# ronin-gw/PyMaSC

Measured on AMD Instinct MI355X. Metric: shifts*genome-bp/sec (whole node), hg38 max_shift=1000; HBM-BW fraction, higher is better.
Workload: dtype u64

## Files before the change

### pymasc_amd/csrc/kernels_events.h

```cpp
#pragma once

#define EV_NQ 2u
#define EV_TBW (EV_NQ * SP_TBW)
#define EV_TB (EV_NQ * SP_TB)
#define EV_LO 64u
#define EV_LO_MAX 512u
#define EV_HI 36u
#ifndef EV_CAPF
#define EV_CAPF 768u
#endif
#ifndef EV_CAPR
#define EV_CAPR 1000u
#endif
#ifndef EV_CAPE_SMALL
#define EV_CAPE_SMALL 1536u
#endif
#define EV_CAPE(BIG) ((BIG) ? 384u : EV_CAPE_SMALL)
#ifndef EV_POOL_SMALL
#define EV_POOL_SMALL 2416u
#endif
#define EV_POOL_ENTRIES(HAS_M, BIG) ((BIG) ? EV_CAPF + EV_CAPR + ((HAS_M) ? 384u : 0u) : ((HAS_M) ? EV_POOL_SMALL : EV_CAPF + EV_CAPR + EV_CAPE_SMALL))
#define EV_RANK_BITS 13u
#ifndef EV_POOL_DEEP
#define EV_POOL_DEEP 4328u
#endif
#define EV_POS 0x1ffffu
#define EV_PAD 12u
#define EV_RSENT 0x3fffffffu
#define EV_JOBSUM(jobstat) (reinterpret_cast<unsigned long long *>((jobstat) + 4 * SP_MAXJOBS))
#define EV_STAT_BYTES (4 * SP_MAXJOBS * sizeof(u32) + 6 * SP_MAXJOBS * sizeof(unsigned long long))
#define EV_SEG_ROWS 6u
#define EV_MAX_SHIFT 8191u
#ifndef EV_PRIO_STAGE
#define EV_PRIO_STAGE 3
#endif
#ifndef EV_PRIO_EVENTS
#define EV_PRIO_EVENTS 2
#endif
#ifndef EV_PRIO_EDGES
#define EV_PRIO_EDGES 1
#endif
#ifndef EV_EDGE_ROLES
#define EV_EDGE_ROLES 1
#endif
#ifndef EV_PAIR_SLOT
#define EV_PAIR_SLOT(w) (w)
#endif
#ifndef EV_ROLE_F
#define EV_ROLE_F 1
#define EV_ROLE_A 2
#define EV_ROLE_B0 3
#define EV_ROLE_B1 0
#endif
#ifndef EV_WAVES
#define EV_WAVES 5
#endif
#ifndef EV_WAVES_NCC
#define EV_WAVES_NCC 8
#endif

#ifdef EV_STAMPS
#define EV_NSTAMP 12
#define EV_STAMP(i)                                                                                    \
    {                                                                                                  \
        unsigned long long t_;                                                                         \
        __builtin_amdgcn_sched_barrier(0);                                                             \
        asm volatile("s_memtime %0\n\ts_waitcnt lgkmcnt(0)" : "=s"(t_)::"memory");                     \
        __builtin_amdgcn_sched_barrier(0);                                                             \
        stamp_acc[i] += t_ - stamp_last;                                                               \
        stamp_last = t_;                                                                               \
    }
#else
#define EV_STAMP(i)
#endif

template <bool HAS_M, bool BIG, bool DEEP = false>
struct EvLds {
    static constexpr u32 LF = 0;
    static constexpr u32 POOL = DEEP ? EV_POOL_DEEP : EV_POOL_ENTRIES(HAS_M, BIG);
    static_assert(POOL + 3 * EV_PAD < (1u << EV_RANK_BITS), "rank field of the forward entries");
    static constexpr u32 WT = LF + POOL + 3 * EV_PAD;
    static constexpr u32 MISC = WT + 32;
    static constexpr u32 IDXF = MISC + 16;
    static constexpr u32 IDXR = IDXF + (HAS_M ? 66u : 0u);
    static constexpr u32 MT0 = IDXR + (HAS_M ? 66u : 0u);
    static_assert(MT0 % 4 == 0, "alignment of the 16-byte stores");
    __host__ __device__ static constexpr u32 sg_words(u32 lo, u32 hi = EV_HI) { return MT0 + (HAS_M ? 4u + lo + EV_TBW + hi : 0u); }
    __host__ __device__ static constexpr u32 row_words(u32 hn) { return BIG ? hn / 2 : hn; }
    __host__ __device__ static constexpr u32 o_gf(u32 hn) { return hn; }
    __host__ __device__ static constexpr u32 o_gr(u32 hn) { return o_gf(hn) + (HAS_M ? row_words(hn) : 0u); }
    __host__ __device__ static constexpr u32 o_ee(u32 hn) { return o_gf(hn); }
    __host__ __device__ static constexpr u32 o_dump(u32 hn) { return o_gr(hn) + (HAS_M ? row_words(hn) : 0u); }
    __host__ __device__ static constexpr u32 o_xch(u32 hn) { return o_dump(hn) + 64; }
    __host__ __device__ static constexpr u32 o_sg(u32 hn) { return o_xch(hn) + 16; }
    __host__ __device__ static constexpr u32 total(u32 hn, u32 lo, u32 nsg, u32 hi = EV_HI) { return o_sg(hn) + nsg * sg_words(lo, hi); }
};

struct EvRegs {
    uint4 f[EV_NQ], r[EV_NQ], m[EV_NQ], h;
    u32 wb[EV_NQ], hbw;
};

template <bool BIG>
__device__ __forceinline__ bool ev_role_mlo(u32 tid, u32 lo) { return BIG ? tid < (lo >> 2) : (tid >> 6) == 1 && (tid & 63u) < 16; }
template <bool BIG>
__device__ __forceinline__ u32 ev_role_mlo_index(u32 tid) { return BIG ? tid : (tid & 63u); }

#ifndef EV_BIG_NT
#define EV_BIG_NT 1
#endif
typedef u32 ev_v4u __attribute__((ext_vector_type(4)));
template <bool GUARD, bool NT>
__device__ __forceinline__ uint4 ev_ld_body(const u32 *__restrict__ p, int64_t j, uint64_t nbits)
{
    if (GUARD || !NT) return ld_quad<GUARD>(p, j, nbits);
    const ev_v4u v = __builtin_nontemporal_load(reinterpret_cast<const ev_v4u *>(p + j));
    return make_uint4(v.x, v.y, v.z, v.w);
}

template <bool HAS_M, bool GUARD, bool BIG>
__device__ __forceinline__ void ev_fetch(EvRegs &er, const u32 *__restrict__ F, const u32 *__restrict__ R,
                                         const u32 *__restrict__ M, int64_t d0, uint64_t nbits, u32 tid, u32 nhr, u32 lo,
                                         bool skip_reads, u32 nhm = EV_HI / 4u)
{
    if (skip_reads) nhr = 0;
#pragma unroll
    for (u32 q = 0; q < EV_NQ; q++) {
        const int64_t j = d0 + (int64_t)q * SP_TBW + 4 * (int64_t)tid;
        if (skip_reads) {
            er.f[q] = make_uint4(0, 0, 0, 0);
            er.r[q] = make_uint4(0, 0, 0, 0);
        } else {
            er.f[q] = ev_ld_body<GUARD, BIG && EV_BIG_NT>(F, j, nbits);
            er.r[q] = ev_ld_body<GUARD, BIG && EV_BIG_NT>(R, j, nbits);
        }
        if (HAS_M) {
            er.m[q] = ev_ld_body<GUARD, BIG && EV_BIG_NT>(M, j, nbits);
            const int64_t j0 = d0 + (int64_t)q * SP_TBW + 4 * (int64_t)(tid & ~63u) - 1;
            er.wb[q] = GUARD ? ld_dword_guarded(M, j0, nbits) : M[j0];
        } else {
            er.m[q] = make_uint4(0, 0, 0, 0);
            er.wb[q] = 0;
        }
    }
    const u32 ht = tid & 63u, hw = tid >> 6;
    const bool m_lo = HAS_M && ev_role_mlo<BIG>(tid, lo), m_hi = HAS_M && hw == 2 && ht < nhm, r_hi = hw == 3 && ht < nhr;
    const u32 *hp = (m_lo || m_hi || skip_reads) ? M : R;
    int64_t jh = d0 + 4 * (int64_t)tid;
    if (m_lo) jh = d0 - (int64_t)lo + 4 * (int64_t)ev_role_mlo_index<BIG>(tid);
    if (m_hi || r_hi) jh = d0 + EV_TBW + 4 * (int64_t)ht;
    er.h = ld_quad<GUARD>(hp, jh, nbits);
    er.hbw = 0;
    if (HAS_M) {
        const bool lo_wave = BIG ? hw < 2 : hw == 1;
        const int64_t jh0 = (lo_wave ? d0 - (int64_t)lo + (BIG ? 256 * (int64_t)hw : 0) : d0 + EV_TBW) - 1;
        er.hbw = GUARD ? ld_dword_guarded(M, jh0, nbits) : M[jh0];
    }
}

template <bool HAS_M>
__device__ __forceinline__ void ev_fetch_fast(EvRegs &er, const SpJobRegs &jb, u32 local_tile, u32 tid, u32 wave, u32 nhr)
{
    const size_t tb = (size_t)local_tile * (EV_TBW * 4u);
    const char *fb = reinterpret_cast<const char *>(jb.F) + tb;
    const char *rb = reinterpret_cast<const char *>(jb.R) + tb;
    const char *mb = reinterpret_cast<const char *>(jb.M) + tb;
    const u32 voff = 16u * tid, lane = tid & 63u;
#pragma unroll
    for (u32 q = 0; q < EV_NQ; q++) {
        const u32 vq = voff + q * (SP_TBW * 4u);
        er.f[q] = *reinterpret_cast<const uint4 *>(fb + vq);
        er.r[q] = *reinterpret_cast<const uint4 *>(rb + vq);
        if (HAS_M) {
            er.m[q] = *reinterpret_cast<const uint4 *>(mb + vq);
            const int32_t sq = (int32_t)(q * (SP_TBW * 4u) + wave * 1024u) - 4;
            er.wb[q] = *reinterpret_cast<const u32 *>(mb + sq);
        } else {
            er.m[q] = make_uint4(0, 0, 0, 0);
            er.wb[q] = 0;
        }
    }
    const char *hb = (HAS_M && wave == 1) ? mb - EV_LO * 4u : (HAS_M && wave == 2) ? mb + EV_TBW * 4u : wave == 3 ? rb + EV_TBW * 4u : rb;
    const u32 lim = (HAS_M && wave == 1) ? 63u : (HAS_M && wave == 2) ? 8u : wave == 3 ? nhr - 1u : 63u;
    const u32 vh = 16u * (lane < lim ? lane : lim);
    er.h = *reinterpret_cast<const uint4 *>(hb + vh);
    er.hbw = HAS_M ? *reinterpret_cast<const u32 *>(hb - 4) : 0u;
}

template <bool HAS_M, bool BIG>
__device__ __forceinline__ void ev_fetch_job(EvRegs &er, const SpJobRegs &jb, u32 local_tile, u32 tid, u32 nhr, u32 lo,
                                             bool skip_reads = false, u32 wave = 0, u32 hi_dwords = EV_HI)
{
    const int64_t d0 = (int64_t)local_tile * EV_TBW;
    const int64_t low = d0 - (int64_t)lo - 1;
    const u32 above = (BIG && 4 * nhr > hi_dwords) ? 4 * nhr : hi_dwords;
    const uint64_t hi = (uint64_t)d0 + EV_TBW + above;
    const bool interior = jb.aligned16 && low >= 0 && hi + 2 <= jb.nbits / 32;
#ifndef EV_NO_FAST_FETCH
    if (!BIG && interior && !skip_reads)
        ev_fetch_fast<HAS_M>(er, jb, local_tile, tid, wave, nhr);
    else
#endif
    if (interior)
        ev_fetch<HAS_M, false, BIG>(er, jb.F, jb.R, jb.M, d0, jb.nbits, tid, nhr, lo, skip_reads, hi_dwords / 4u);
    else
        ev_fetch<HAS_M, true, BIG>(er, jb.F, jb.R, jb.M, d0, jb.nbits, tid, nhr, lo, skip_reads, hi_dwords / 4u);
}

__device__ __forceinline__ void ev_emit_f(const uint4 f, const uint4 r, const uint4 m, u32 idx, u32 rank0, u32 base_bit,
                                          u32 *list)
{
    const u64 fs[2] = {(u64)f.x | ((u64)f.y << 32), (u64)f.z | ((u64)f.w << 32)};
    const u64 rs[2] = {(u64)r.x | ((u64)r.y << 32), (u64)r.z | ((u64)r.w << 32)};
    const u64 ms[2] = {(u64)m.x | ((u64)m.y << 32), (u64)m.z | ((u64)m.w << 32)};
    u32 rk = rank0;
#pragma unroll
    for (u32 k = 0; k < 2; k++) {
        u64 ww = fs[k];
        while (ww) {
            const u32 b = (u32)__builtin_ctzll(ww);
            ww &= ww - 1;
            const u64 below = (rs[k] << (63u - b)) << 1;
            list[idx] = (base_bit + 64u * k + b) | ((rk + (u32)__popcll(below)) << 17) | ((u32)((ms[k] >> b) & 1ull) << 31);
            idx++;
        }
        rk += (u32)__popcll(rs[k]);
    }
}
__device__ __forceinline__ void ev_emit_pos(const uint4 v, u32 idx, u32 base_bit, u32 *list)
{
    const u64 vs[2] = {(u64)v.x | ((u64)v.y << 32), (u64)v.z | ((u64)v.w << 32)};
#pragma unroll
    for (u32 k = 0; k < 2; k++) {
        u64 ww = vs[k];
        while (ww) {
            const u32 b = (u32)__builtin_ctzll(ww);
            ww &= ww - 1;
            list[idx] = base_bit + 64u * k + b;
            idx++;
        }
    }
}

__device__ __forceinline__ u32 ev_below(u32 last_dword, u32 first)
{
    return (u32)__builtin_amdgcn_update_dpp((int)first, (int)last_dword, 0x138, 0xf, 0xf, false);
}

__device__ __forceinline__ u32 ev_mbit(const u32 *MT, u32 q) { return (MT[q >> 5] >> (q & 31u)) & 1u; }

template <bool BIG>
__device__ __forceinline__ void ev_add_cell(u32 *row, u32 cell, u32 val)
{
    if (BIG)
        atomicAdd(&row[cell >> 1], val << ((cell & 1u) << 4));
    else
        atomicAdd(&row[cell], val);
}

__device__ __forceinline__ void ev_zero_row5(u32 *__restrict__ slab, u32 segment, u32 hn, u32 gt, u32 nt)
{
    u32 *row = slab + ((size_t)segment * EV_SEG_ROWS + 5u) * hn;
    for (u32 i = gt; i < hn; i += nt) row[i] = 0u;
    asm volatile("s_waitcnt vmcnt(0)" ::: "memory");
}

template <bool HAS_M, bool DO_NCC, bool DO_MLEN, u32 NSG, bool BIG, typename JT = SpJobTable, bool DEEP = false>
__global__ void __launch_bounds__(256 * NSG, BIG ? 4 : (HAS_M ? (DEEP ? 4 : EV_WAVES) : EV_WAVES_NCC))
k_cc_events(const JT jobs, u32 njobs, u32 total_tiles, u32 tiles_per_wg, u32 c, u32 S, u32 nhr, u32 max_lag,
            u32 hn_arg, u32 lo_arg, u32 hi_arg, u32 *__restrict__ slab, unsigned char *__restrict__ tile_flags,
            unsigned char *__restrict__ tile_flags_ac, u32 *__restrict__ n_flagged, u32 *__restrict__ jobstat)
{
    typedef EvLds<HAS_M, BIG, DEEP> L;
    static_assert(!DEEP || (HAS_M && !BIG), "DEEP: the max_shift <= 1023 instantiations with a track");
    static_assert(BIG || NSG == 1, "the max_shift <= 1023 instantiations are one sub-group per workgroup");
    constexpr u32 NT = 256 * NSG;
    extern __shared__ __align__(16) u32 ev_dyn_lds[];
    __shared__ __align__(16) u32 ev_static_lds[BIG ? 4 : L::total(1024, EV_LO, 1)];
    u32 *const lds = BIG ? ev_dyn_lds : ev_static_lds;
    const u32 HN = BIG ? hn_arg : 1024u;
    const u32 LO = BIG ? lo_arg : EV_LO;
    const u32 HI = BIG ? (hi_arg & 0xffffu) : EV_HI;
    const bool EE_LDS = BIG && DO_MLEN && (hi_arg >> 16) != 0;
    const u32 BIAS = LO * 32u;
    const u32 sg = NSG > 1 ? __builtin_amdgcn_readfirstlane(threadIdx.x >> 8) : 0u;
    u32 *const hN = lds;
    u32 *const hGF = lds + L::o_gf(HN);
    u32 *const hGR = lds + L::o_gr(HN);
    u32 *const hEE = lds + L::o_ee(HN);
    u32 *const xch = lds + L::o_xch(HN);
    u32 *const sgb = lds + L::o_sg(HN) + sg * L::sg_words(LO, HI);
    u32 *const hEEb = lds + L::total(HN, LO, NSG, HI);
    u32 *const MT = sgb + L::MT0 + 4;
    unsigned short *const idxF = reinterpret_cast<unsigned short *>(sgb + L::IDXF);
    unsigned short *const idxR = reinterpret_cast<unsigned short *>(sgb + L::IDXR);
    u32 *const LF = sgb + L::LF;
    u32 *const wt = sgb + L::WT;

    const u32 gt = threadIdx.x;
    const u32 tid_ = NSG > 1 ? (threadIdx.x & 255u) : threadIdx.x;
    const u32 wave = __builtin_amdgcn_readfirstlane(tid_ >> 6);
    const u32 g0 = blockIdx.x * tiles_per_wg;
    const u32 g1 = g0 + tiles_per_wg < total_tiles ? g0 + tiles_per_wg : total_tiles;
    if (g0 >= g1) return;
    {
#pragma nounroll
        for (u32 i = gt; i < L::o_sg(HN); i += NT) lds[i] = 0;
        if (EE_LDS)
            for (u32 i = gt; i < HN / 2; i += NT) hEEb[i] = 0;
    }

    FIRST_JOB(ji, JT, jobs, njobs, g0)
    u32 jn = ji;
    if (BIG && DO_MLEN && !EE_LDS) ev_zero_row5(slab, blockIdx.x + ji, HN, gt, NT);
    EvRegs er;
    SpJobRegs pj;
    load_job(pj, jobs.j[ji]);
    bool act_var = true;
    if (NSG > 1) {
        const u32 lim = pj.tile_end < g1 ? pj.tile_end : g1;
        act_var = g0 + sg < lim;
    }
    if (NSG == 1 || act_var) ev_fetch_job<HAS_M, BIG>(er, pj, g0 + sg - pj.tile0, tid_, nhr, LO, false, wave, HI);
    u32 job_mode = 0;
    u32 unreported = 0;
    bool had_dense = false;
    bool cur_skip = false, next_skip = false;
    u32 cur_tile0 = pj.tile0, cur_flag0 = pj.flag0;
    u32 cntB = 0, cnt0 = 0;
    u32 cntM = 0, cntU = 0;
    u32 accF = 0, accR = 0, accE = 0;
    bool seg_written = false;
    bool seg_gr_written = false;
#ifdef EV_STAMPS
    unsigned long long stamp_acc[EV_NSTAMP] = {0, 0, 0, 0, 0, 0, 0, 0, 0, 0, 0, 0};
    unsigned long long stamp_last;
    asm volatile("s_memtime %0\n\ts_waitcnt lgkmcnt(0)" : "=s"(stamp_last)::"memory");
#endif

    for (u32 g = g0; g < g1;) {
        const bool act = NSG == 1 ? true : act_var;
        EV_STAMP(9)
        __syncthreads();
        EV_STAMP(0)
        if (EV_PRIO_STAGE) __builtin_amdgcn_s_setprio(EV_PRIO_STAGE);
        u32 tid = tid_;
        asm volatile("" : "+v"(tid));
        const u32 lane = tid & 63;
        u32 cF[EV_NQ] = {0, 0}, cR[EV_NQ] = {0, 0}, cE[EV_NQ] = {0, 0}, cEh = 0, cRh = 0, pendM = 0, pendU = 0;
        const bool h_below = HAS_M && ev_role_mlo<BIG>(tid, LO), h_above = HAS_M && wave == 2 && lane < HI / 4u;
        const u32 hb = ev_role_mlo_index<BIG>(tid);
        const bool h_r = wave == 3 && lane < nhr;
        u32 pF = 0, pR = 0, pE = 0, pH = 0, sF = 0, sR = 0, sH = 0, sE = 0, sX = 0;
        if (act) {
#pragma unroll
            for (u32 q = 0; q < EV_NQ; q++) {
                cF[q] = popc4(er.f[q]);
                cR[q] = popc4(er.r[q]);
                if (HAS_M) {
                    const u32 bel = ev_below(er.m[q].w, er.wb[q]);
                    cE[q] = popc4(edge_words(er.m[q], bel));
                    *reinterpret_cast<uint4 *>(MT + LO + q * SP_TBW + 4 * tid) = er.m[q];
                    if (DO_MLEN) {
                        pendM += popc4(er.m[q]);
                        pendU += (cE[q] + (er.m[q].w >> 31) - (bel >> 31)) >> 1;
                    }
                }
            }
            const u32 hbel = HAS_M ? ev_below(er.h.w, er.hbw) : 0u;
            if (h_below || h_above) {
                cEh = popc4(edge_words(er.h, hbel));
                *reinterpret_cast<uint4 *>(MT + (h_below ? 4 * hb : LO + EV_TBW + 4 * lane)) = er.h;
                if (h_below && hb == 0) MT[-1] = er.hbw;
            }
            if (h_r) cRh = popc4(er.h);
            pF = cF[0] | (cF[1] << 16);
            pR = cR[0] | (cR[1] << 16);
            pE = cE[0] | (cE[1] << 16);
            pH = h_below ? cEh : cEh << 16;
            sF = pF;
            sR = pR;
            sH = cRh;
            sE = pE;
            sX = pH;
            if (HAS_M)
                wave_inclusive_scan5(sF, sR, sH, sE, sX);
            else
                wave_inclusive_scan3(sF, sR, sH);
            if (lane == 63) {
                wt[0 + wave] = sF;
                wt[4 + wave] = sR;
                wt[8 + wave] = sH;
                if (HAS_M) {
                    wt[12 + wave] = sE;
                    wt[16 + wave] = sX;
                }
            }
        }
        EV_STAMP(1)
        __syncthreads();
        EV_STAMP(2)
        u32 nF = 0, nRt = 0, nR = 0, nE = 0, TXb = 0, TE0 = 0, TE1 = 0;
        bool dense = false, do_edges = false;
        u32 *LR = LF, *LE = LF;
        u32 gnext = g + NSG;
        if (act) {
            u32 bF = 0, bR = 0, bH = 0, bE = 0, bX = 0, tF = 0, tR = 0, tH = 0, tE = 0, tX = 0;
#pragma unroll
            for (u32 w = 0; w < 4; w++) {
                const u32 xF = wt[w], xR = wt[4 + w], xH = wt[8 + w], xE = HAS_M ? wt[12 + w] : 0u, xX = HAS_M ? wt[16 + w] : 0u;
                if (w < wave) {
                    bF += xF;
                    bR += xR;
                    bH += xH;
                    bE += xE;
                    bX += xX;
                }
                tF += xF;
                tR += xR;
                tH += xH;
                tE += xE;
                tX += xX;
            }
            const u32 TF0 = tF & 0xffffu, TR0 = tR & 0xffffu;
            TE0 = tE & 0xffffu;
            TE1 = tE >> 16;
            TXb = tX & 0xffffu;
            nF = __builtin_amdgcn_readfirstlane(TF0 + (tF >> 16));
            nRt = __builtin_amdgcn_readfirstlane(TR0 + (tR >> 16));
            nR = __builtin_amdgcn_readfirstlane(nRt + tH);
            nE = __builtin_amdgcn_readfirstlane(TXb + TE0 + TE1 + (tX >> 16));
            const bool dense_e = HAS_M && nE > EV_CAPE(BIG);
            const bool dense_r = cur_skip || (BIG ? (nF > EV_CAPF || nR > EV_CAPR)
                                                  : nF + nR + ((HAS_M && !dense_e) ? nE : 0u) > L::POOL);
            dense = dense_e || dense_r;
            do_edges = HAS_M && !dense_e && (!dense || DO_MLEN);
            LR = LF + (dense ? 0u : nF) + EV_PAD;
            LE = LR + (dense ? 0u : nR) + EV_PAD;
            const u32 my_tile = g + sg;
            if (!dense) {
                const u32 eF = bF + sF - pF, eR = bR + sR - pR;
                const u32 oR0 = eR & 0xffffu, oR1 = TR0 + (eR >> 16);
                ev_emit_f(er.f[0], er.r[0], er.m[0], eF & 0xffffu, oR0, BIAS + 0 * SP_TB + 128u * tid, LF);
                ev_emit_f(er.f[1], er.r[1], er.m[1], TF0 + (eF >> 16), oR1, BIAS + 1 * SP_TB + 128u * tid, LF);
                ev_emit_pos(er.r[0], oR0, BIAS + 0 * SP_TB + 128u * tid, LR);
                ev_emit_pos(er.r[1], oR1, BIAS + 1 * SP_TB + 128u * tid, LR);
                if (h_r) ev_emit_pos(er.h, nRt + bH + sH - cRh, BIAS + EV_TB + 128u * lane, LR);
                if (tid < EV_PAD) LR[nR + tid] = EV_RSENT;
                else if (HAS_M && tid < 2 * EV_PAD) LF[nF + tid - EV_PAD] = EV_POS;
                if (HAS_M) {
                    if ((tid & 3u) == 0) {
                        idxF[tid >> 2] = (unsigned short)(eF & 0xffffu);
                        idxF[64 + (tid >> 2)] = (unsigned short)(TF0 + (eF >> 16));
                        idxR[tid >> 2] = (unsigned short)oR0;
                        idxR[64 + (tid >> 2)] = (unsigned short)oR1;
                    }
                    if (tid == 255) {
// ... 174 lines not shown
                        const u32 m0 = MT[q0 >> 5], m1 = MT[q1 >> 5];
                        atomicAdd(&hN[a0], (DO_NCC ? 1u : 0u) | (((m0 >> (q0 & 31u)) << 16) & flm));
                        atomicAdd(&hN[a1], (DO_NCC ? 1u : 0u) | (((m1 >> (q1 & 31u)) << 16) & flm));
                    } else {
                        atomicAdd(&hN[a0], 1u);
                        atomicAdd(&hN[a1], 1u);
                    }
                    d0 = y0 - x;
                    d1 = y1 - x;
                    h0 = d0 <= S;
                    h1 = d1 <= S;
                } while (__ballot(h0));
            }
#endif
            EV_STAMP(6)
#ifndef EV_ABL_NOREV
            if (HAS_M)
                for (u32 b = (wave + 2) & 3; b < nbR; b += 4) {
                    const u32 i = 64 * b + lane;
                    if (i < nRt) {
                        const u32 p = LR[i];
                        cnt0 += ev_mbit(MT, p) & ev_mbit(MT, p + c);
                    }
                }
#endif
            EV_STAMP(8)
            if (EV_PRIO_EDGES != EV_PRIO_EVENTS) __builtin_amdgcn_s_setprio(EV_PRIO_EDGES);
#ifndef EV_ABL_NOFE
            const u32 nEv = (HAS_M && BIG && DO_MLEN && HI > EV_HI) ? __builtin_amdgcn_readfirstlane(sgb[L::MISC + 1]) : nE;
            if (HAS_M)
                for (u32 eb = 0; eb < nEv; eb += 64) {
                    const u32 i = eb + lane;
                    const bool in = i < nEv;
                    const u32 ee = in ? LE[i] : 0u;
                    const int32_t j = (int32_t)(ee & EV_POS);
                    const u32 sgn = (u32)(((int32_t)ee >> 31) | 1);
                    const int32_t tile_end = (int32_t)(BIAS + EV_TB);
#if EV_EDGE_ROLES
                    const bool roleF = wave == EV_ROLE_F, roleA = wave == EV_ROLE_A, roleB = wave == EV_ROLE_B0 || wave == EV_ROLE_B1;
                    const u32 woffF = 0, wstrF = 1, woffA = 0, wstrA = 1;
                    const u32 wstrB = EV_ROLE_B0 == EV_ROLE_B1 ? 1u : 2u, woffB = (EV_ROLE_B0 != EV_ROLE_B1 && wave == EV_ROLE_B1) ? 1u : 0u;
#else
                    const bool roleF = true, roleA = true, roleB = true;
                    const u32 woffF = wave, wstrF = 4, woffA = wave, wstrA = 4, woffB = wave, wstrB = 4;
#endif
                    if (roleF) {
                        const int32_t lo = j - (int32_t)c;
                        const u32 span = in ? S : 0u;
                        int32_t bb = (lo - (int32_t)BIAS) >> 9;
                        bb = bb < 0 ? 0 : (bb > 128 ? 128 : bb);
                        u32 idx = (u32)idxF[bb] + woffF;
                        u32 e0 = LF[idx], e1 = LF[idx + wstrF];
                        u32 u0 = (e0 & EV_POS) - (u32)lo, u1 = (e1 & EV_POS) - (u32)lo;
                        bool more = (int32_t)u0 < (int32_t)span;
                        if (__ballot(more)) do {
                            const bool h0 = u0 < span && (e0 >> 31) != 0, h1 = u1 < span && (e1 >> 31) != 0;
                            ev_add_cell<BIG>(hGF, h0 ? u0 + 1 : dumpGF, sgn);
                            ev_add_cell<BIG>(hGF, h1 ? u1 + 1 : dumpGF, sgn);
                            idx = more ? idx + 2 * wstrF : idx;
                            e0 = LF[idx];
                            e1 = LF[idx + wstrF];
                            u0 = (e0 & EV_POS) - (u32)lo;
                            u1 = (e1 & EV_POS) - (u32)lo;
                            more = (int32_t)u0 < (int32_t)span;
                        } while (__ballot(more));
                    }
#pragma unroll
                    for (u32 kind = 0; kind < 2; kind++) {
                        if (!(kind == 0 ? roleA : roleB)) continue;
                        const u32 woff = kind == 0 ? woffA : woffB, wstr = kind == 0 ? wstrA : wstrB;
                        const int32_t lo = kind == 0 ? j : j - (int32_t)c;
                        int32_t sp = tile_end - lo;
                        const int32_t full = kind == 0 ? (int32_t)S : 2 * (int32_t)S;
                        sp = sp < full ? sp : full;
                        const u32 span = (in && sp > 0) ? (u32)sp : 0u;
                        int32_t bb = (lo - (int32_t)BIAS) >> 9;
                        bb = bb < 0 ? 0 : (bb > 128 ? 128 : bb);
                        u32 idx = (u32)idxR[bb] + woff;
                        u32 p0 = LR[idx], p1 = LR[idx + wstr];
                        u32 u0 = p0 - (u32)lo, u1 = p1 - (u32)lo;
                        bool more = (int32_t)u0 < (int32_t)span;
                        if (__ballot(more)) do {
                            const bool h0 = u0 < span, h1 = u1 < span;
                            const u32 d0 = kind == 0 ? u0 + 1 : (u0 + 2) >> 1, d1 = kind == 0 ? u1 + 1 : (u1 + 2) >> 1;
                            const u32 q0 = h0 ? (kind == 0 ? p0 + c - 2 * d0 : p0 - d0 + 1) : BIAS;
                            const u32 q1 = h1 ? (kind == 0 ? p1 + c - 2 * d1 : p1 - d1 + 1) : BIAS;
                            const u32 m0 = MT[q0 >> 5], m1 = MT[q1 >> 5];
                            idx = more ? idx + 2 * wstr : idx;
                            p0 = LR[idx];
                            p1 = LR[idx + wstr];
                            ev_add_cell<BIG>(hGR, h0 ? d0 : dumpGR, (0u - sgn) * ((m0 >> (q0 & 31u)) & 1u));
                            ev_add_cell<BIG>(hGR, h1 ? d1 : dumpGR, (0u - sgn) * ((m1 >> (q1 & 31u)) & 1u));
                            u0 = p0 - (u32)lo;
                            u1 = p1 - (u32)lo;
                            more = (int32_t)u0 < (int32_t)span;
                        } while (__ballot(more));
                    }
                }
#endif
        }
        {
            if (!BIG && DO_MLEN && do_edges) {
                const u32 dumpEE = L::o_dump(HN) - L::o_ee(HN) + lane;
                const u32 nEt = TE0 + TE1;
                for (u32 b = (wave + 1) & 3; 64 * b < nEt; b += 4) {
                    const u32 i = 64 * b + lane;
                    const bool in = i < nEt;
                    const u32 ent = in ? LE[TXb + i] : 0u;
                    const u32 pos = ent & EV_POS, hi = pos + max_lag;
                    u32 e = in ? TXb + i + 1 : nE;
                    u32 e0 = LE[e], e1 = LE[e + 1];
                    u32 p0 = e0 & EV_POS, p1 = e1 & EV_POS;
                    bool h0 = p0 <= hi, h1 = p1 <= hi;
                    if (__ballot(h0)) do {
                        atomicAdd(&hEE[h0 ? p0 - pos : dumpEE], (u32)(((int32_t)(e0 ^ ent) >> 31) | 1) << 16);
                        atomicAdd(&hEE[h1 ? p1 - pos : dumpEE], (u32)(((int32_t)(e1 ^ ent) >> 31) | 1) << 16);
                        e = h1 ? e + 2 : nE;
                        e0 = LE[e];
                        e1 = LE[e + 1];
                        p0 = e0 & EV_POS;
                        p1 = e1 & EV_POS;
                        h0 = p0 <= hi;
                        h1 = p1 <= hi;
                    } while (__ballot(h0));
                }
            }
        }
        if (EV_PRIO_EVENTS) __builtin_amdgcn_s_setprio(0);
        EV_STAMP(7)
        if (NSG == 1) {
            if (!dense) {
                accF += nF;
                accR += nRt;
            }
            if (DO_MLEN && do_edges) accE += nE;
        } else {
#pragma unroll
            for (u32 k = 0; k < NSG; k++) {
                const u32 v = xch[k];
                accF += v & 0xffffu;
                accR += v >> 16;
                if (DO_MLEN) accE += xch[4 + k];
            }
            accF = __builtin_amdgcn_readfirstlane(accF);
            accR = __builtin_amdgcn_readfirstlane(accR);
            accE = __builtin_amdgcn_readfirstlane(accE);
        }
        const bool leaving = jn != ji || gnext >= g1;
        const bool risk = HAS_M && (BIG ? (accF + NSG * EV_CAPF > 32767u || 3u * (accR + NSG * EV_CAPR) > 32767u ||
                                           (EE_LDS && accE + NSG * L::POOL > 32767u))
                                        : (accF + L::POOL > 32767u || (DO_MLEN && accE + EV_CAPE(BIG) > 32767u)));
        if (NSG == 1 && leaving && tid == 0) {
            const u32 pc = xch[14], pa = xch[15];
            if (pc) atomicAdd(n_flagged, pc);
            if (pa) atomicAdd(n_flagged + 1, pa);
            xch[14] = 0;
            xch[15] = 0;
        }
#ifndef EV_NO_GR_FLUSH
        const bool risk_gr_only = BIG && HAS_M && !leaving && risk && !(accF + NSG * EV_CAPF > 32767u) &&
                                  !(EE_LDS && accE + NSG * L::POOL > 32767u);
#else
        const bool risk_gr_only = false;
#endif
        if (risk_gr_only) {
            __syncthreads();
            u32 *seg = slab + (size_t)(blockIdx.x + ji) * EV_SEG_ROWS * HN;
            const bool add = seg_gr_written;
#pragma nounroll
            for (u32 k = gt; k < (HN >> 1); k += NT) {
                const u32 w = hGR[k];
                hGR[k] = 0;
                const int32_t lo16 = (int32_t)(short)(w & 0xffffu);
                const int32_t hi16 = (int32_t)(short)((w - (u32)lo16) >> 16);
                uint2 *dst = reinterpret_cast<uint2 *>(seg + (size_t)3 * HN + 2 * k);
                uint2 v = make_uint2((u32)lo16, (u32)hi16);
                if (add) {
                    const uint2 o = *dst;
                    v.x += o.x;
                    v.y += o.y;
                }
                *dst = v;
            }
            accR = 0;
            seg_gr_written = true;
        } else if (leaving || risk) {
            __syncthreads();
            u32 *seg = slab + (size_t)(blockIdx.x + ji) * EV_SEG_ROWS * HN;
            const bool add = seg_written;
#pragma nounroll
            for (u32 i = gt; i < HN; i += NT) {
                const u32 w = hN[i];
                hN[i] = 0;
                if (HAS_M) {
                    const u32 lo16 = w & 0xffffu, hi16 = w >> 16;
                    seg[i] = add ? seg[i] + lo16 : lo16;
                    seg[2 * HN + i] = add ? seg[2 * HN + i] + hi16 : hi16;
                } else {
                    seg[i] = add ? seg[i] + w : w;
                }
            }
            if (HAS_M) {
                if (BIG) {
#pragma nounroll
                    for (u32 i = gt; i < HN; i += NT) {
                        const u32 half = HN >> 1, row = i >= half ? 1u : 0u, k = i - row * half;
                        u32 *src = (row ? hGR : hGF) + k;
                        const u32 w = *src;
                        *src = 0;
                        const int32_t lo16 = (int32_t)(short)(w & 0xffffu);
                        const int32_t hi16 = (int32_t)(short)((w - (u32)lo16) >> 16);
                        uint2 *dst = reinterpret_cast<uint2 *>(seg + (size_t)(row ? 3 : 1) * HN + 2 * k);
                        uint2 v = make_uint2((u32)lo16, (u32)hi16);
                        if (row ? seg_gr_written : add) {
                            const uint2 o = *dst;
                            v.x += o.x;
                            v.y += o.y;
                        }
                        *dst = v;
                    }
                    if (DO_MLEN && EE_LDS) {
#pragma nounroll
                        for (u32 k = gt; k < HN / 2; k += NT) {
                            const u32 w = hEEb[k];
                            hEEb[k] = 0;
                            const int32_t lo16 = (int32_t)(short)(w & 0xffffu);
                            const int32_t hi16 = (int32_t)(short)((w - (u32)lo16) >> 16);
                            uint2 *dst = reinterpret_cast<uint2 *>(seg + (size_t)5 * HN + 2 * k);
                            uint2 v = make_uint2((u32)lo16, (u32)hi16);
                            if (add) {
                                const uint2 o = *dst;
                                v.x += o.x;
                                v.y += o.y;
                            }
                            *dst = v;
                        }
                    }
                } else {
                    {
                        u32 v[4] = {cntB, cnt0, cntM, cntU};
#pragma unroll
                        for (u32 k = 0; k < 4; k++)
                            for (int off = 32; off > 0; off >>= 1) v[k] += __shfl_down(v[k], off, 64);
                        if ((gt & 63u) == 0) {
#pragma unroll
                            for (u32 k = 0; k < 4; k++)
                                if (k < 2 || DO_MLEN) atomicAdd(&xch[8 + 2 + k], v[k]);
                        }
                        cntB = cnt0 = cntM = cntU = 0;
                    }
                    __syncthreads();
                    const u32 a0 = xch[8 + 4], runs = xch[8 + 5];
                    const u32 k0 = 4 * gt;
                    const uint4 wgf = *reinterpret_cast<const uint4 *>(hGF + k0), wgr = *reinterpret_cast<const uint4 *>(hGF + 1024 + k0);
                    const u32 cgf[4] = {wgf.x, wgf.y, wgf.z, wgf.w}, cgr[4] = {wgr.x, wgr.y, wgr.z, wgr.w};
                    u32 pgf[4], pgr[4], dl[4], tGF = 0, tGR = 0, tX = 0;
#pragma unroll
                    for (u32 j = 0; j < 4; j++) {
                        const int32_t lo16 = (int32_t)(short)(cgf[j] & 0xffffu);
                        const int32_t ee = (int32_t)(short)((cgf[j] - (u32)lo16) >> 16);
                        tGF += (u32)lo16;
                        tGR += cgr[j];
                        tX += (k0 + j == 0) ? 0u - runs : 0u - (u32)ee;
                        pgf[j] = tGF;
                        pgr[j] = tGR;
                        dl[j] = tX;
                    }
                    u32 sGF = tGF, sGR = tGR, sX = tX;
                    wave_inclusive_scan3(sGF, sGR, sX);
                    if ((gt & 63u) == 63u) {
                        wt[0 + (gt >> 6)] = sGF;
                        wt[4 + (gt >> 6)] = sGR;
                        wt[8 + (gt >> 6)] = sX;
                    }
                    __syncthreads();
                    u32 bGF = sGF - tGF, bGR = sGR - tGR, bX = sX - tX;
                    for (u32 w = 0; w < (gt >> 6); w++) {
                        bGF += wt[w];
                        bGR += wt[4 + w];
                        bX += wt[8 + w];
                    }
                    u32 tD = 0, ex[4];
#pragma unroll
                    for (u32 j = 0; j < 4; j++) {
                        pgf[j] += bGF;
                        pgr[j] += bGR;
                        dl[j] += bX;
                        ex[j] = tD;
                        tD += dl[j];
                    }
                    {
                        uint4 *d1 = reinterpret_cast<uint4 *>(seg + 1 * 1024 + k0), *d3 = reinterpret_cast<uint4 *>(seg + 3 * 1024 + k0);
                        uint4 v1 = make_uint4(pgf[0], pgf[1], pgf[2], pgf[3]), v3 = make_uint4(pgr[0], pgr[1], pgr[2], pgr[3]);
                        if (add) {
                            const uint4 o1 = *d1, o3 = *d3;
                            v1.x += o1.x; v1.y += o1.y; v1.z += o1.z; v1.w += o1.w;
                            v3.x += o3.x; v3.y += o3.y; v3.z += o3.z; v3.w += o3.w;
                        }
                        *d1 = v1;
                        *d3 = v3;
                    }
                    if (DO_MLEN) {
                        u32 sD = wave_inclusive_scan(tD);
                        __syncthreads();
                        if ((gt & 63u) == 63u) wt[12 + (gt >> 6)] = sD;
                        __syncthreads();
                        u32 bD = sD - tD;
                        for (u32 w = 0; w < (gt >> 6); w++) bD += wt[12 + w];
                        *reinterpret_cast<uint4 *>(hGF + k0) = make_uint4(a0 + bD + ex[0], a0 + bD + ex[1], a0 + bD + ex[2], a0 + bD + ex[3]);
                        __syncthreads();
#pragma unroll
                        for (u32 j = 0; j < 4; j++) {
                            const u32 d = k0 + j;
                            if (d <= S) {
                                const int32_t k = (int32_t)c - (int32_t)d;
                                const u32 av = hGF[k < 0 ? -k : k];
                                u32 *de = seg + (size_t)5 * 1024 + d;
                                *de = add ? *de + av : av;
                            }
                        }
                        __syncthreads();
                    }
                    *reinterpret_cast<uint4 *>(hGF + k0) = make_uint4(0, 0, 0, 0);
                    *reinterpret_cast<uint4 *>(hGF + 1024 + k0) = make_uint4(0, 0, 0, 0);
                    if (gt < 6) {
                        const u32 v = xch[8 + gt];
                        u32 *ds = seg + 4 * HN + gt;
                        *ds = add ? *ds + v : v;
                        if (v) atomicAdd(EV_JOBSUM(jobstat) + 6 * ji + gt, (unsigned long long)v);
                    }
                    __syncthreads();
                    if (gt < 6) xch[8 + gt] = 0;
                }
            }
            accF = 0;
            accR = 0;
            accE = 0;
            seg_written = true;
            seg_gr_written = true;
            if (leaving && !(!BIG && HAS_M)) {
                u32 v[6] = {0, 0, cntB, cnt0, cntM, cntU};
#pragma unroll
                for (u32 k = 2; k < 6; k++)
                    for (int off = 32; off > 0; off >>= 1) v[k] += __shfl_down(v[k], off, 64);
                if ((gt & 63u) == 0) {
#pragma unroll
                    for (u32 k = 2; k < 6; k++)
                        if (k < 4 || DO_MLEN) atomicAdd(&xch[8 + k], v[k]);
                }

                __syncthreads();
                if (gt < 6) {
                    const u32 v = xch[8 + gt];
                    seg[4 * HN + gt] = v;
                    if (!BIG && v) atomicAdd(EV_JOBSUM(jobstat) + 6 * ji + gt, (unsigned long long)v);
                    xch[8 + gt] = 0;
                }
                cntB = 0;
                cnt0 = 0;
                cntM = 0;
                cntU = 0;
            }
            if (leaving) {
                seg_written = false;
                seg_gr_written = false;
            }
        }
        if (jn != ji) {
            if (BIG && DO_MLEN && !EE_LDS) ev_zero_row5(slab, blockIdx.x + jn, HN, gt, NT);
            job_mode = 0;
            next_skip = false;
            unreported = 0;
            if (had_dense && tid_ == 0) sgb[L::MISC] = 0;
            had_dense = false;
        }
        cur_skip = fetched_skip;
        ji = jn;
        cur_tile0 = pj.tile0;
        cur_flag0 = pj.flag0;
        g = gnext;
    }
#ifdef EV_STAMPS
    if ((gt & 63) == 0) {
        unsigned long long *dbg = reinterpret_cast<unsigned long long *>(slab + (size_t)(gridDim.x + njobs) * EV_SEG_ROWS * HN);
        for (int i = 0; i < EV_NSTAMP; i++) dbg[((size_t)blockIdx.x * 4 * NSG + (gt >> 6)) * EV_NSTAMP + i] = stamp_acc[i];
    }
#endif
}

#define EVF_TASKS 6u
#define EVF_CHUNKS 8u
struct EvFinishArgs {
    const u32 *slab;
    const unsigned long long *jobsum;
    u32 S, out_stride, has_m, do_ncc, fused_mlen, zero_mlen, keep_scalar2;
    uint4 *zero_area;
    u32 zero_quads;
};

__global__ void __launch_bounds__(1024)
k_events_finish(const SpJobTable jobs, u32 njobs, const EvFinishArgs a, const PlanLaunch pcc, const PlanLaunch pac)
{
    __shared__ u32 acc[128];
    const u32 tid = threadIdx.x, chunk = blockIdx.x, task = blockIdx.y, job = blockIdx.z;
    if (job == njobs) {
        const u32 id = task * EVF_CHUNKS + chunk, nid = EVF_TASKS * EVF_CHUNKS;
        if (id == 0) plan_flagged(pcc);
        else if (id == 1) plan_flagged(pac);
        else
            for (u32 i = (id - 2) * 1024 + tid; i < a.zero_quads; i += (nid - 2) * 1024) a.zero_area[i] = make_uint4(0, 0, 0, 0);
        return;
    }
    const SpJobDev &jb = jobs.j[job];
    const u32 S = a.S, n = S + 1;
    u64 *const out = jb.out;
    const size_t os = a.out_stride;
    const unsigned long long *js = a.jobsum + 6 * job;
    if (task == 0) {
        if (chunk != 0) return;
        u64 *dst = out + (size_t)PMX_ROW_SCALARS * os;
        for (u32 k = tid; k < a.out_stride; k += 1024) {
            if (k == 2 && a.keep_scalar2 && !a.fused_mlen) continue;
            dst[k] = k < 2 ? js[k] : (k == 2 ? (a.fused_mlen ? js[4] : 0ull) : (k == 3 && jb.tile_first == 0 ? (u64)PMX_PATH_SPARSE : 0ull));
        }
        return;
    }
    const u32 dst_row = task == 1 ? PMX_ROW_NCC_CCBINS : task == 2 ? PMX_ROW_MSCC_CCBINS : task == 3 ? PMX_ROW_MSCC_FSUM
                        : task == 4 ? PMX_ROW_MSCC_RSUM : PMX_ROW_MLEN;
    const bool produced = task == 1 ? a.do_ncc != 0 : task == 5 ? a.fused_mlen != 0 : a.has_m != 0;
    const u32 col0 = 128 * chunk;
    u64 *dst = out + (size_t)dst_row * os;
    if (!produced) {
        if (task != 5 || !a.has_m || a.zero_mlen)
            for (u32 k = col0 + tid; k < a.out_stride && k < col0 + 128; k += 1024) dst[k] = 0;
        if (chunk == EVF_CHUNKS - 1 && (task != 5 || !a.has_m || a.zero_mlen))
            for (u32 k = 128 * EVF_CHUNKS + tid; k < a.out_stride; k += 1024) dst[k] = 0;
        return;
    }
    if (col0 >= n) return;
    const u32 src_row = task == 1 ? 0u : task == 2 ? 2u : task == 3 ? 1u : task == 4 ? 3u : 5u;
    if (tid < 128) acc[tid] = 0;
    __syncthreads();
    const u32 q = tid & 31u, g = tid >> 5;
    const size_t stride = (size_t)EV_SEG_ROWS * 1024;
    const u32 *p = a.slab + (size_t)job * stride + (size_t)src_row * 1024 + col0 + 4 * q;
    u32 s0 = 0, s1 = 0, s2 = 0, s3 = 0;
    for (u32 w = jb.wg_first + g; w <= jb.wg_last; w += 32) {
        const uint4 v = *reinterpret_cast<const uint4 *>(p + (size_t)w * stride);
        s0 += v.x;
        s1 += v.y;
        s2 += v.z;
        s3 += v.w;
    }
    atomicAdd(&acc[4 * q + 0], s0);
    atomicAdd(&acc[4 * q + 1], s1);
    atomicAdd(&acc[4 * q + 2], s2);
    atomicAdd(&acc[4 * q + 3], s3);
    __syncthreads();
    if (tid < 128 && col0 + tid < n) {
        const u32 t = acc[tid];
        dst[col0 + tid] = task == 3 ? (u64)(u32)((u32)js[2] - t) : task == 4 ? (u64)(u32)((u32)js[3] + t) : (u64)t;
    }
}

struct EvTailPlan {
    u32 cc_first[SP_MAXJOBS], cc_last[SP_MAXJOBS];
    u32 ac_first[SP_MAXJOBS], ac_last[SP_MAXJOBS];
};

#define EV_TAIL_THREADS 1024u
template <typename JT = SpJobTable>
__global__ void __launch_bounds__(EV_TAIL_THREADS)
k_events_tail(const u32 *__restrict__ slab, const JT jobs, const EvTailPlan plan, const u32 *__restrict__ slab_cc,
              const u32 *__restrict__ slab_ac, const u32 *__restrict__ n_flagged, u32 S, u32 out_stride, u32 has_m, u32 do_ncc,
              u32 max_lag, u32 lagcap, int32_t c, u32 fused, u32 rowlen, u32 slow_path, const u32 *__restrict__ plan_cc,
              const u32 *__restrict__ plan_ac, u32 prefix_done)
{
    __shared__ long long part[256];
    __shared__ long long tot[2];
    const u32 job = blockIdx.x, tid = threadIdx.x;
    const SpJobDev &jb = jobs.j[job];
    const bool flagged = slow_path && n_flagged[blockIdx.y == 1 ? 1 : 0] != 0;
    if ((blockIdx.y >= 2 && !flagged) || (blockIdx.y == 1 && !fused)) return;
    if (prefix_done && !flagged) return;
    if (blockIdx.y == 1) {
        if (flagged) {
            u64 *P = jb.out2, *N = jb.out2 + lagcap, *scal = jb.out2 + 2 * (size_t)lagcap;
            const size_t stride = (size_t)AC_SEG_ROWS * 1024;
            const u32 i0 = plan_ac ? plan_ac[PLAN_JOBWG + 2 * job] : plan.ac_first[job];
            const u32 i1 = plan_ac ? plan_ac[PLAN_JOBWG + 2 * job + 1] : plan.ac_last[job] + 1;
            for (u32 k = tid; k <= max_lag; k += EV_TAIL_THREADS) {
                u64 sp = 0, sn = 0;
#pragma unroll 4
                for (u32 i = i0; i < i1; i++) {
                    const u32 w = plan_ac ? plan_ac[PLAN_LIST + i] : i;
                    const u32 *seg = slab_ac + (size_t)(w + job) * stride;
                    sp += seg[k];
                    sn += seg[1024 + k];
                }
                P[k] = prefix_done ? sp : P[k] + sp;
                N[k] = prefix_done ? sn : N[k] + sn;
            }
            if (tid < 2) {
                u64 sc = 0;
                for (u32 i = i0; i < i1; i++) {
                    const u32 w = plan_ac ? plan_ac[PLAN_LIST + i] : i;
                    sc += slab_ac[(size_t)(w + job) * stride + 2 * 1024 + tid];
                }
                scal[tid] = prefix_done ? sc : scal[tid] + sc;
            }
            __threadfence_block();
            __syncthreads();
        }
        autocorr_finish_job(jb, part, max_lag, lagcap, prefix_done ? 2u : 1u, c, S, out_stride, EV_TAIL_THREADS);
        return;
    }
    if (has_m && blockIdx.y == 0 && !prefix_done) {
        long long bf = 0, r0 = 0;
        for (u32 w = jb.wg_first + tid; w <= jb.wg_last; w += EV_TAIL_THREADS) {
            const u32 *sc = slab + ((size_t)(w + job) * EV_SEG_ROWS + 4) * rowlen;
            bf += sc[2];
            r0 += sc[3];
        }
        const long long eb = block_exclusive_offset(bf, part, tid);
        if (tid == EV_TAIL_THREADS - 1) tot[0] = eb + bf;
        const long long e0 = block_exclusive_offset(r0, part, tid);
        if (tid == EV_TAIL_THREADS - 1) tot[1] = e0 + r0;
        __syncthreads();
        const long long Bf = tot[0], R0 = tot[1];
        const u32 seg = (S + 1 + EV_TAIL_THREADS - 1) / EV_TAIL_THREADS;
        const u32 k0 = tid * seg, k1 = (k0 + seg < S + 1) ? k0 + seg : S + 1;
#pragma unroll
        for (u32 row = 0; row < 2; row++) {
            long long *v = reinterpret_cast<long long *>(jb.out + (size_t)(row ? PMX_ROW_MSCC_RSUM : PMX_ROW_MSCC_FSUM) * out_stride);
            long long sum = 0;
            for (u32 k = k0; k < k1; k++) sum += v[k];
            long long run = block_exclusive_offset(sum, part, tid);
            for (u32 k = k0; k < k1; k++) {
                run += v[k];
                v[k] = row ? R0 + run : Bf - run;
            }
            __syncthreads();
        }
    }
    if (flagged) {
        const u32 dst_row[4] = {PMX_ROW_NCC_CCBINS, PMX_ROW_MSCC_FSUM, PMX_ROW_MSCC_CCBINS, PMX_ROW_MSCC_RSUM};
        const size_t stride = (size_t)SP_SEG_ROWS * 1024;
        const u32 i0 = plan_cc ? plan_cc[PLAN_JOBWG + 2 * job] : plan.cc_first[job];
        const u32 i1 = plan_cc ? plan_cc[PLAN_JOBWG + 2 * job + 1] : plan.cc_last[job] + 1;
        for (u32 r = 0; r < 4; r++) {
            if (r == 0 ? !do_ncc : !has_m) continue;
            if (blockIdx.y != (r == 0 ? 2u : (r == 2 ? 3u : 0u))) continue;
            u64 *dst = jb.out + (size_t)dst_row[r] * out_stride;
            for (u32 d = tid; d <= S; d += EV_TAIL_THREADS) {
                u64 sum = 0;
#pragma unroll 4
                for (u32 i = i0; i < i1; i++) {
                    const u32 w = plan_cc ? plan_cc[PLAN_LIST + i] : i;
                    sum += slab_cc[(size_t)(w + job) * stride + r * 1024 + d];
                }
                dst[d] += sum;
            }
        }
        if (blockIdx.y == 2 && tid < 2) {
            u64 sc = 0;
            for (u32 i = i0; i < i1; i++) {
                const u32 w = plan_cc ? plan_cc[PLAN_LIST + i] : i;
                sc += slab_cc[(size_t)(w + job) * stride + 4 * 1024 + tid];
            }
            jb.out[(size_t)PMX_ROW_SCALARS * out_stride + tid] += sc;
        }
    }
}
```

### pymasc_amd/csrc/kernels_sparse.hip

```cpp
#include "pmx_common.h"

#include <stdio.h>
#include <string.h>
#include <type_traits>
#include <vector>

#define SP_TB 32768u
#define SP_TBW 1024u
#define SP_RHI 36u
#define SP_MLO 68u
#define SP_MHI 36u
#define SP_MW (SP_MLO + SP_TBW + SP_MHI)
#define SP_HALO_M (SP_MLO * 32u)
#define SP_CAP 512u
#define SP_NP 11
#define SP_NQ 11
#define SP_QLIMIT 511u
#ifndef SP_QSOFT
#define SP_QSOFT 256u
#endif
#define SP_NS 16
#define SP_NL 24
#define SP_L2LIMIT (1u << 21)
#define SP_MAXJOBS 32u
// ... 403 lines not shown
    g.slot = wave * spw + (lane >> lgG);
    g.l4 = 4u * (lane & ((1u << lgG) - 1));
    g.quad_span = g.total_slots * 4;
    g.lg_span = 10 - lgG;
    g.lg_region = lgG + 1;
    return g;
}

__device__ __forceinline__ u32 emit_reserve(const uint4 w, u32 *cursor)
{
    const u32 n = __popc(w.x) + __popc(w.y) + __popc(w.z) + __popc(w.w);
    return n ? atomicAdd(cursor, n) : 0u;
}

template <bool WIDE = false, bool CHECKED = true>
__device__ __forceinline__ void emit_positions(const uint4 w, const uint4 flag_bits, u32 idx0, u32 round_lo, u32 *list, u32 tid,
                                               u32 base = 0)
{
    u32 id = idx0 - round_lo;
    if (!WIDE) {
    const u32 ws[4] = {w.x, w.y, w.z, w.w};
    const u32 fs[4] = {flag_bits.x, flag_bits.y, flag_bits.z, flag_bits.w};
#pragma unroll
    for (u32 k = 0; k < 4; k++) {
        u32 ww = ws[k];
        while (ww) {
            const u32 b = __builtin_ctz(ww);
            ww &= ww - 1;
            if (!CHECKED || id < SP_CAP) list[id] = (base + 128u * tid + 32u * k + b) | (((fs[k] >> b) & 1u) << 16);
            id++;
        }
    }
    } else {
    const u64 ws[2] = {(u64)w.x | ((u64)w.y << 32), (u64)w.z | ((u64)w.w << 32)};
    const u64 fs[2] = {(u64)flag_bits.x | ((u64)flag_bits.y << 32), (u64)flag_bits.z | ((u64)flag_bits.w << 32)};
#pragma unroll
    for (u32 k = 0; k < 2; k++) {
        u64 ww = ws[k];
        while (ww) {
            const u32 b = (u32)__builtin_ctzll(ww);
            ww &= ww - 1;
            if (!CHECKED || id < SP_CAP) list[id] = (base + 128u * tid + 64u * k + b) | ((u32)((fs[k] >> b) & 1ull) << 16);
            id++;
        }
    }
    }
}

template <bool WIDE>
__device__ __forceinline__ void emit_positions_round0(const uint4 w, const uint4 flag_bits, u32 idx0, u32 *list, u32 tid)
{
#ifdef SP_EMIT_CHECKED
    emit_positions<WIDE, true>(w, flag_bits, idx0, 0, list, tid);
#else
    const u32 n = __popc(w.x) + __popc(w.y) + __popc(w.z) + __popc(w.w);
    if (idx0 + n <= SP_CAP)
        emit_positions<WIDE, false>(w, flag_bits, idx0, 0, list, tid);
    else
        emit_positions<WIDE, true>(w, flag_bits, idx0, 0, list, tid);
#endif
}

template <bool HAS_M>
__device__ __forceinline__ void build_forward_records(u32 *lds, uint4 *recs, u32 qbase, u32 qstride, u32 lane_in_slot,
                                                      u32 G, u32 nq, u32 n, int32_t c)
{
    typedef SpLds<HAS_M> L;
    const u32 *pl = lds + L::PLF;
    for (u32 j = lane_in_slot; j < 4 * nq; j += G) {
        uint4 rec = make_uint4(0u, L::ZERO * 4u, (L::ZERO + 32u) * 4u, 0u);
        const u32 idx = 4u * (qbase + (j >> 2) * qstride) + (j & 3u);
        if (idx < n) {
            const u32 e = pl[idx];
            const u32 pos = e & 0x7fffu;
            rec.x = pos;
            rec.y = (L::R + (pos >> 5)) * 4u;
            if (HAS_M) {
                const u32 a0 = pos + (u32)c + SP_HALO_M - 31u;
                rec.w = a0;
                if (e >> 16) rec.z = (L::M + (a0 >> 5)) * 4u;
            }
        }
        recs[j] = rec;
    }
}

__device__ __forceinline__ void build_reverse_records(u32 *lds, uint4 *recs, u32 qbase, u32 qstride, u32 lane_in_slot, u32 G,
                                                      u32 nq, u32 n, int32_t c)
{
    typedef SpLds<true> L;
    const u32 *pl = lds + L::PLR;
    for (u32 j = lane_in_slot; j < 4 * nq; j += G) {
        uint4 rec = make_uint4(0u, (L::ZERO + 32u) * 4u, (L::ZERO + 32u) * 4u, 0u);
        const u32 idx = 4u * (qbase + (j >> 2) * qstride) + (j & 3u);
        if (idx < n) {
            const u32 p = pl[idx] & 0x7fffu;
            const u32 a1 = p + SP_HALO_M - 31u;
            const u32 bb = p + SP_HALO_M + (u32)c;
            const u32 a2 = (bb >> 1) - 31u;
            rec.x = a1;
            rec.y = (L::M + (a1 >> 5)) * 4u;
            rec.z = (((bb & 1u) ? L::O : L::E) + (a2 >> 5)) * 4u;
            rec.w = a2;
        }
        recs[j] = rec;
    }
}

__device__ __forceinline__ u32 lds_window(const u32 *lds, u32 byte_addr, u32 shift_word)
{
    const u32 *p = reinterpret_cast<const u32 *>(reinterpret_cast<const char *>(lds) + byte_addr);
    return __builtin_amdgcn_alignbit(p[1], p[0], shift_word);
}

#ifdef SP_STAMPS
#define SP_NSTAMP 12
#define SP_STAMP(i)                                                                                    \
    {                                                                                                  \
        unsigned long long t_;                                                                         \
        __builtin_amdgcn_sched_barrier(0);                                                             \
        asm volatile("s_memtime %0\n\ts_waitcnt lgkmcnt(0)" : "=s"(t_)::"memory");                     \
        __builtin_amdgcn_sched_barrier(0);                                                             \
        stamp_acc[i] += t_ - stamp_last;                                                               \
        stamp_last = t_;                                                                               \
    }
#else
#define SP_STAMP(i)
#endif

#ifndef SP_WAVES
#define SP_WAVES 3
#endif
#ifndef SP_WAVES_CH
#define SP_WAVES_CH 3
#endif
#ifndef SP_WAVES_CH_NCC
#define SP_WAVES_CH_NCC 6
#endif
#ifndef SP_WAVES_NCC
#define SP_WAVES_NCC 6
#endif
#ifndef SP_PRIO_STAGE
#define SP_PRIO_STAGE 3
#endif
#ifndef SP_PRIO_PROCESS
#define SP_PRIO_PROCESS 2
#endif
#ifndef SP_ROLES
#define SP_ROLES 0
#endif
template <bool HAS_M, bool DO_NCC, bool CH, typename JT>
__device__ __forceinline__ void cc_sparse_body(u32 *const lds, const u32 bx, const JT &jobs, u32 njobs, u32 total_tiles, u32 tiles_per_wg,
                                               int32_t c, u32 lgG, u32 *__restrict__ slab, const unsigned char *__restrict__ tile_flags,
                                               const u32 *__restrict__ plan, u32 add_stride)
{
    typedef SpLds<HAS_M> L;
    u32 *const cursor = lds + L::MISC;
    u32 *const acc = lds + L::ACC;
    u32 *const stage = lds + L::STAGE;

    const u32 tid = threadIdx.x;
    const SlotGeom sg = slot_geom(lgG, tid);

    const u32 g0 = plan ? plan[2 * bx] : bx * tiles_per_wg;
    const u32 g1 = plan ? plan[2 * bx + 1] : (g0 + tiles_per_wg < total_tiles ? g0 + tiles_per_wg : total_tiles);
    if (g0 >= g1) return;

    for (u32 i = tid; i < 40; i += 256) lds[L::ZERO + i] = 0;
    for (u32 i = tid; i < L::NCOUNTERS * SP_NL * 32; i += 256) acc[i] = 0;

    constexpr bool ROLES = SP_ROLES && HAS_M && DO_NCC && !CH;
#ifdef SP_NOPAIRS
    constexpr bool QUAD_PAIRS = false;
#else
    constexpr bool QUAD_PAIRS = !HAS_M;
#endif
    constexpr u32 RCAP = ROLES ? SP_CAP / 2 : SP_CAP;
    Planes cN, cF, cC, cR;
    planes_zero(cN);
    planes_zero(cF);
    planes_zero(cC);
    planes_zero(cR);
    Planes c0, c1;
    planes_zero(c0);
    planes_zero(c1);
    u32 qF = 0, qR = 0;
    u32 qFw = 0, qRw = 0;
    const u32 wave = __builtin_amdgcn_readfirstlane(threadIdx.x >> 6);
    u32 q2 = 0;
    u32 totF = 0, totR = 0;
    u32 cntR_thread = 0;
    bool seg_written = false;

    FIRST_JOB(ji, JT, jobs, njobs, g0)

#ifdef SP_STAMPS
    unsigned long long stamp_acc[SP_NSTAMP] = {0, 0, 0, 0, 0, 0, 0, 0, 0, 0, 0, 0};
    unsigned long long stamp_last;
    asm volatile("s_memtime %0\n\ts_waitcnt lgkmcnt(0)" : "=s"(stamp_last)::"memory");
#endif
    TileRegs tr;
    TileRegsX tx;
    SpJobRegs pj;
    load_job(pj, jobs.j[ji]);
    tile_fetch_job<HAS_M, CH>(tr, tx, pj, g0 - pj.tile0, tid, tile_flags);
    if (tid < 4) cursor[tid] = 0;
    u32 par = 0;
    const u32 G = 1u << lgG;
    const u32 lane_in_slot = sg.l4 >> 2;

    u32 g = g0, gnext = g0, round_lo = 0, jn = ji;
    u32 nF = 0, nR = 0, iF = 0, iR = 0, nmax = 0, pendR = 0;
    bool leaving = false;
    u32 leave_job = 0;
    for (;;) {
        const bool have_tile = g < g1;
        SP_STAMP(7)
        __syncthreads();
        SP_STAMP(0)
        if (have_tile && round_lo == 0) {
            if (SP_PRIO_STAGE) __builtin_amdgcn_s_setprio(SP_PRIO_STAGE);
#ifdef SP_RESERVE_LATE
            tile_store<HAS_M, CH>(tr, tx, lds, tid);
            SP_STAMP(2)
#endif
            if (!HAS_M) pendR = __popc(tr.r.x) + __popc(tr.r.y) + __popc(tr.r.z) + __popc(tr.r.w);
            iF = emit_reserve(tr.f, &cursor[2 * par]);
            SP_STAMP(8)
            if (HAS_M) iR = emit_reserve(tr.r, &cursor[2 * par + 1]);
            SP_STAMP(9)
#ifndef SP_RESERVE_LATE
            tile_store<HAS_M, CH>(tr, tx, lds, tid);
            SP_STAMP(2)
#endif
#ifndef SP_ABL_NOEMIT
            emit_positions_round0<HAS_M>(tr.f, HAS_M ? tr.m : tr.f, iF, lds + L::PLF, tid);
            SP_STAMP(10)
            if (HAS_M) emit_positions_round0<HAS_M>(tr.r, tr.r, iR, lds + L::PLR, tid);
#endif
            if (tid < 2) cursor[2 * (par ^ 1) + tid] = 0;
            SP_STAMP(3)
            gnext = g + 1;
            if (tile_flags) {
                const u32 lim = pj.tile_end < g1 ? pj.tile_end : g1;
                gnext = pj.tile0 + next_flagged_tile(tile_flags + pj.flag0, gnext - pj.tile0, lim - pj.tile0);
            }
            if (gnext < g1) {
                if (gnext >= pj.tile_end) {
                    jn = ji + 1;
                    load_job(pj, jobs.j[jn]);
                }
                tile_fetch_job<HAS_M, CH>(tr, tx, pj, gnext - pj.tile0, tid, tile_flags);
            }
            SP_STAMP(4)
            if (SP_PRIO_STAGE) __builtin_amdgcn_s_setprio(0);
            __syncthreads();
            SP_STAMP(5)
#ifdef SP_ABL_NOPROC
            nF = 0;
            nR = 0;
#else
            nF = cursor[2 * par];
            nR = HAS_M ? cursor[2 * par + 1] : 0u;
#endif
            par ^= 1;
            nmax = nF > nR ? nF : nR;
        } else if (have_tile) {
            TileRegs cur;
            TileRegsX curx;
            tile_fetch<HAS_M, false, true>(cur, curx, jobs.j[ji].F, jobs.j[ji].R, jobs.j[ji].M,
                                           (int64_t)(g - jobs.j[ji].tile0) * SP_TBW, 0, jobs.j[ji].nbits, tid);
            emit_positions(cur.f, HAS_M ? cur.m : cur.f, iF, round_lo, lds + L::PLF, tid);
            if (HAS_M) emit_positions(cur.r, cur.r, iR, round_lo, lds + L::PLR, tid);
            __syncthreads();
        }
        u32 nFr = 0, nRr = 0;
        if (have_tile) {
            nFr = nF > round_lo ? (nF - round_lo < RCAP ? nF - round_lo : RCAP) : 0u;
            nRr = nR > round_lo ? (nR - round_lo < RCAP ? nR - round_lo : RCAP) : 0u;
        }
        const u32 lg_spw = 6 - lgG;
        const u32 wiF = (((nFr + 3) >> 2) + (1u << lg_spw) - 1) >> lg_spw, wiR = (((nRr + 3) >> 2) + (1u << lg_spw) - 1) >> lg_spw;
        const bool roleA = wave < 2;
        const u32 wr = ROLES ? (wave & 1u) : wave;
        const u32 nqF = ROLES ? (wiF + 1) >> 1 : (wiF + 3) >> 2;
        const u32 nqR = ROLES ? (wiR + 1) >> 1 : (wiR + 3) >> 2;
#ifdef SP_UNBALANCED
        const u32 nqFw = nqF, nqRw = nqR, wrR = wr;
#else
        const u32 nqFw = wr < wiF ? (ROLES ? (wiF - wr + 1) >> 1 : (wiF - wr + 3) >> 2) : 0u;
#ifdef SP_RDEAL_SAME
        const u32 wrR = wr;
#else
        const u32 wrR = ROLES ? wr : 3u - wave;
#endif
        const u32 nqRw = (ROLES && roleA) ? 0u : (wrR < wiR ? (ROLES ? (wiR - wrR + 1) >> 1 : (wiR - wrR + 3) >> 2) : 0u);
#endif
        const u32 rslotR = (wrR << lg_spw) + (sg.slot & ((1u << lg_spw) - 1));

        if (leaving || (round_lo == 0 && (qF >= SP_QSOFT || qR >= SP_QSOFT)) || qF + nqF > SP_QLIMIT ||
            qR + nqR > SP_QLIMIT) {
            if (ROLES) {
                counter_to_lds(c0, qFw, lgG, tid, stage, acc, roleA);
                counter_to_lds(c0, qFw, lgG, tid, stage, acc + 1 * SP_NL * 32, !roleA);
                counter_to_lds(c1, qFw, lgG, tid, stage, acc + 2 * SP_NL * 32, roleA);
                counter_to_lds(c1, qRw, lgG, tid, stage, acc + 3 * SP_NL * 32, !roleA);
            } else {
                if (DO_NCC) counter_to_lds(cN, qFw, lgG, tid, stage, acc);
                if (HAS_M) {
                    counter_to_lds(cF, qFw, lgG, tid, stage, acc + 1 * SP_NL * 32);
                    counter_to_lds(cC, qFw, lgG, tid, stage, acc + 2 * SP_NL * 32);
                    counter_to_lds(cR, qRw, lgG, tid, stage, acc + 3 * SP_NL * 32);
                }
            }
            q2 += (qF > qR ? qF : qR) * 4u * sg.total_slots;
            qF = 0;
            qR = 0;
            qFw = 0;
// ... 314 lines not shown
            for (u32 w = jb.wg_first; w <= jb.wg_last; w++) sum += (u64)(long long)(int32_t)p[(size_t)(w + job) * stride + i];
        else
            for (u32 w = jb.wg_first; w <= jb.wg_last; w++) sum += p[(size_t)(w + job) * stride + i];
        u64 *dst = rs.use_out2 ? jb.out2 + (size_t)rs.dst_row[r] + jb.d_off + i
                               : jb.out + (size_t)rs.dst_row[r] * rs.out_stride + jb.d_off + i;
        *dst = rs.accumulate ? *dst + sum : sum;
    }
    return true;
}

template <typename JT>
__device__ __forceinline__ void reduce_segments_row(const u32 *__restrict__ slab, const JT &jobs, u32 seg_rows,
                                                    const ReduceSpec &rs, const u32 *__restrict__ gate, u32 r)
{
    __shared__ u64 part[32][32];
    if (gate && *gate == 0 && rs.accumulate) return;
    if ((!gate || *gate != 0) && reduce_segments_row_wide(slab, jobs, seg_rows, rs, r)) return;
    for (u32 bx = blockIdx.x; bx < rs_rowlen(rs) / 32; bx += gridDim.x) {
        reduce_segments_chunk(slab, jobs, seg_rows, rs, gate, r, bx, part);
        __syncthreads();
    }
}

template <typename JT = SpJobTable>
__global__ void __launch_bounds__(256)
k_reduce_segments(const u32 *__restrict__ slab, const JT jobs, u32 seg_rows, ReduceSpec rs,
                  const u32 *__restrict__ gate)
{
    reduce_segments_row(slab, jobs, seg_rows, rs, gate, blockIdx.y);
}

__global__ void __launch_bounds__(1024)
k_reduce_segments2(const u32 *__restrict__ slab, const SpJobTable jobs, u32 seg_rows, ReduceSpec rsA, ReduceSpec rsB)
{
    const u32 rowsA = rsA.nrows + rsA.nzero;
    if (blockIdx.y < rowsA)
        reduce_segments_row(slab, jobs, seg_rows, rsA, nullptr, blockIdx.y);
    else
        reduce_segments_row(slab, jobs, seg_rows, rsB, nullptr, blockIdx.y - rowsA);
}

#ifndef AC_NQ
#define AC_NQ 2
#endif
#define AC_TBW (AC_NQ * SP_TBW)
#define AC_TB (AC_NQ * SP_TB)
#define AC_W (AC_TBW + SP_RHI)
struct AcLds {
    static constexpr u32 ZERO = 0;
    static constexpr u32 U = 40;
    static constexpr u32 D = U + AC_W;
    static constexpr u32 PL = D + AC_W;
    static constexpr u32 REC = PL + SP_CAP;
    static constexpr u32 ACC = REC + 4 * SP_CAP;
    static constexpr u32 STAGE = REC;
    static constexpr u32 MISC = ACC + 2 * SP_NL * 32;
    static constexpr u32 TOTAL = MISC + 16;
};
#define AC_SEG_ROWS 3u
#ifndef AC_WAVES
#define AC_WAVES 4
#endif
#ifndef AC_WAVES_CH
#define AC_WAVES_CH 4
#endif

struct AcRegs {
    uint4 m[AC_NQ], h;
    u32 below[AC_NQ];
    u32 hbelow;
    uint4 mw[AC_NQ];
    u32 wbelow[AC_NQ];
};

template <bool GUARD, bool CH>
__device__ __forceinline__ void ac_fetch(AcRegs &ar, const u32 *__restrict__ M, int64_t d0, int64_t off, uint64_t nbits, u32 tid)
{
#pragma unroll
    for (int q = 0; q < AC_NQ; q++) {
        const int64_t j = d0 + (int64_t)q * SP_TBW + 4 * (int64_t)tid;
        ar.m[q] = ld_quad<GUARD>(M, j, nbits);
        ar.below[q] = GUARD ? ld_dword_guarded(M, j - 1, nbits) : M[j - 1];
        if (CH) {
            ar.mw[q] = ld_quad<GUARD>(M, j + off, nbits);
            ar.wbelow[q] = GUARD ? ld_dword_guarded(M, j + off - 1, nbits) : M[j + off - 1];
        }
    }
    ar.h = make_uint4(0, 0, 0, 0);
    ar.hbelow = 0;
    if (tid < 9) {
        const int64_t jh = d0 + off + AC_TBW + 4 * (int64_t)tid;
        ar.h = ld_quad<GUARD>(M, jh, nbits);
        ar.hbelow = GUARD ? ld_dword_guarded(M, jh - 1, nbits) : M[jh - 1];
    }
}

template <bool CH>
__device__ __forceinline__ void ac_fetch_job(AcRegs &ar, const SpJobDev &jb, u32 local_tile, u32 tid,
                                             const unsigned char *__restrict__ flags)
{
    if (flags && !flags[jb.flag0 + local_tile]) {
#pragma unroll
        for (int q = 0; q < AC_NQ; q++) {
            ar.m[q] = make_uint4(0, 0, 0, 0);
            ar.below[q] = 0;
            if (CH) {
                ar.mw[q] = make_uint4(0, 0, 0, 0);
                ar.wbelow[q] = 0;
            }
        }
        ar.h = make_uint4(0, 0, 0, 0);
        ar.hbelow = 0;
        return;
    }
    const int64_t d0 = (int64_t)local_tile * AC_TBW;
    const int64_t off = CH ? (int64_t)(jb.d_off / 32) : 0;
    const uint64_t hi = (uint64_t)(d0 + off) + AC_TBW + SP_RHI;
    const bool interior = jb.aligned16 && local_tile > 0 && hi + 2 <= jb.nbits / 32;
    if (interior)
        ac_fetch<false, CH>(ar, jb.M, d0, off, jb.nbits, tid);
    else
        ac_fetch<true, CH>(ar, jb.M, d0, off, jb.nbits, tid);
}

__device__ __forceinline__ void edge_quad(const uint4 m, u32 below, uint4 &U, uint4 &D)
{
    const u32 s0 = (m.x << 1) | (below >> 31), s1 = (m.y << 1) | (m.x >> 31);
    const u32 s2 = (m.z << 1) | (m.y >> 31), s3 = (m.w << 1) | (m.z >> 31);
    U = make_uint4(m.x & ~s0, m.y & ~s1, m.z & ~s2, m.w & ~s3);
    D = make_uint4(~m.x & s0, ~m.y & s1, ~m.z & s2, ~m.w & s3);
}

__device__ __forceinline__ void build_edge_records(u32 *lds, uint4 *recs, u32 first, u32 lane_in_slot, u32 G, u32 nq, u32 n)
{
    const u32 *pl = lds + AcLds::PL;
    for (u32 j = lane_in_slot; j < 4 * nq; j += G) {
        uint4 rec = make_uint4(0u, AcLds::ZERO * 4u, AcLds::ZERO * 4u, 0u);
        if (first + j < n) {
            const u32 e = pl[first + j];
            const u32 pos = e & 0xffffu;
            const u32 au = (AcLds::U + (pos >> 5)) * 4u, ad = (AcLds::D + (pos >> 5)) * 4u;
            const bool fall = (e >> 16) != 0;
            rec = make_uint4(pos, fall ? ad : au, fall ? au : ad, 0u);
        }
        recs[j] = rec;
    }
}

__device__ __forceinline__ long long block_exclusive_offset(long long local_sum, long long *part, u32 tid);

template <bool CH, typename JT>
__device__ __forceinline__ void autocorr_edges_body(u32 *const lds, const u32 bx, const JT &jobs, u32 njobs, u32 total_tiles, u32 tiles_per_wg,
                                                    u32 lgG, u32 *__restrict__ slab, const unsigned char *__restrict__ tile_flags,
                                                    const u32 *__restrict__ plan, u32 add_stride, int32_t add_c, u32 add_shift, u32 add_lag)
{
    typedef AcLds L;
    u32 *const cursor = lds + L::MISC;
    u32 *const acc = lds + L::ACC;
    u32 *const stage = lds + L::STAGE;

    const u32 tid = threadIdx.x;
    const SlotGeom sg = slot_geom(lgG, tid);

    const u32 g0 = plan ? plan[2 * bx] : bx * tiles_per_wg;
    const u32 g1 = plan ? plan[2 * bx + 1] : (g0 + tiles_per_wg < total_tiles ? g0 + tiles_per_wg : total_tiles);
    if (g0 >= g1) return;

    for (u32 i = tid; i < 40; i += 256) lds[L::ZERO + i] = 0;
    for (u32 i = tid; i < 2 * SP_NL * 32; i += 256) acc[i] = 0;

    Planes cP, cN;
    planes_zero(cP);
    planes_zero(cN);
    u32 qc = 0, q2 = 0;
    u32 cntM = 0, cntU = 0;
    bool seg_written = false;

    FIRST_JOB(ji, JT, jobs, njobs, g0)

    AcRegs ar;
    ac_fetch_job<CH>(ar, jobs.j[ji], g0 - jobs.j[ji].tile0, tid, tile_flags);
    if (tid < 2) cursor[tid] = 0;
    u32 par = 0;
    const u32 G = 1u << lgG;
    const u32 lane_in_slot = sg.l4 >> 2;

    u32 g = g0, gnext = g0, round_lo = 0, jn = ji, n = 0, i0 = 0, pendM = 0, pendU = 0;
    bool leaving = false;
    u32 leave_job = 0;
    for (;;) {
        const bool have_tile = g < g1;
        __syncthreads();
        if (have_tile && round_lo == 0) {
            uint4 E[AC_NQ], Dq[AC_NQ];
            pendM = 0;
            pendU = 0;
            u32 nE = 0;
#pragma unroll
            for (int q = 0; q < AC_NQ; q++) {
                uint4 U, D;
                edge_quad(ar.m[q], ar.below[q], U, D);
                if (CH) {
                    uint4 Uw, Dw;
                    edge_quad(ar.mw[q], ar.wbelow[q], Uw, Dw);
                    reinterpret_cast<uint4 *>(lds + L::U + q * SP_TBW)[tid] = Uw;
                    reinterpret_cast<uint4 *>(lds + L::D + q * SP_TBW)[tid] = Dw;
                } else {
                    reinterpret_cast<uint4 *>(lds + L::U + q * SP_TBW)[tid] = U;
                    reinterpret_cast<uint4 *>(lds + L::D + q * SP_TBW)[tid] = D;
                }
                E[q] = make_uint4(U.x | D.x, U.y | D.y, U.z | D.z, U.w | D.w);
                Dq[q] = D;
                pendM += __popc(ar.m[q].x) + __popc(ar.m[q].y) + __popc(ar.m[q].z) + __popc(ar.m[q].w);
                pendU += __popc(U.x) + __popc(U.y) + __popc(U.z) + __popc(U.w);
                nE += __popc(E[q].x) + __popc(E[q].y) + __popc(E[q].z) + __popc(E[q].w);
            }
            if (tid < 9) {
                uint4 Uh, Dh;
                edge_quad(ar.h, ar.hbelow, Uh, Dh);
                reinterpret_cast<uint4 *>(lds + L::U + AC_TBW)[tid] = Uh;
                reinterpret_cast<uint4 *>(lds + L::D + AC_TBW)[tid] = Dh;
            }
            i0 = nE ? atomicAdd(&cursor[par], nE) : 0u;
            {
                u32 at = i0;
#pragma unroll
                for (int q = 0; q < AC_NQ; q++) {
                    emit_positions(E[q], Dq[q], at, 0, lds + L::PL, tid, q * SP_TB);
                    at += __popc(E[q].x) + __popc(E[q].y) + __popc(E[q].z) + __popc(E[q].w);
                }
            }
            if (tid == 0) cursor[par ^ 1] = 0;
            jn = ji;
            gnext = g + 1;
            if (!CH && tile_flags) {
                const u32 je = jobs.j[ji].tile0 + jobs.j[ji].ntiles, lim = je < g1 ? je : g1;
                gnext = jobs.j[ji].tile0 + next_flagged_tile(tile_flags + jobs.j[ji].flag0, gnext - jobs.j[ji].tile0, lim - jobs.j[ji].tile0);
            }
            if (gnext < g1) {
                if (gnext >= jobs.j[ji].tile0 + jobs.j[ji].ntiles) jn = ji + 1;
                ac_fetch_job<CH>(ar, jobs.j[jn], gnext - jobs.j[jn].tile0, tid, tile_flags);
            }
            __syncthreads();
            n = cursor[par];
            par ^= 1;
        } else if (have_tile) {
            AcRegs cur;
            ac_fetch<true, false>(cur, jobs.j[ji].M, (int64_t)(g - jobs.j[ji].tile0) * AC_TBW, 0, jobs.j[ji].nbits, tid);
            u32 at = i0;
#pragma unroll
            for (int q = 0; q < AC_NQ; q++) {
                uint4 U2, D2;
                edge_quad(cur.m[q], cur.below[q], U2, D2);
                const uint4 E2 = make_uint4(U2.x | D2.x, U2.y | D2.y, U2.z | D2.z, U2.w | D2.w);
                emit_positions(E2, D2, at, round_lo, lds + L::PL, tid, q * SP_TB);
                at += __popc(E2.x) + __popc(E2.y) + __popc(E2.z) + __popc(E2.w);
            }
            __syncthreads();
        }
        u32 nr = 0;
        if (have_tile) nr = n > round_lo ? (n - round_lo < SP_CAP ? n - round_lo : SP_CAP) : 0u;
        const u32 nq = (nr + sg.quad_span - 1) >> sg.lg_span;

        if (leaving || (round_lo == 0 && qc >= SP_QSOFT) || qc + nq > SP_QLIMIT) {
            counter_to_lds(cP, qc, lgG, tid, stage, acc);
            counter_to_lds(cN, qc, lgG, tid, stage, acc + SP_NL * 32);
            q2 += qc * 4u * sg.total_slots;
            qc = 0;
        }
        if (leaving || q2 >= SP_L2LIMIT) {
            const u32 j = leaving ? leave_job : ji;
            u32 *seg = slab + (size_t)(bx + j) * AC_SEG_ROWS * 1024;
            acc_to_segment(acc, 2, 0u, seg, seg_written, tid);
            q2 = 0;
            seg_written = true;
            if (leaving) {
                u32 vm = cntM, vu = cntU;
                for (int off = 32; off > 0; off >>= 1) {
                    vm += __shfl_down(vm, off, 64);
                    vu += __shfl_down(vu, off, 64);
                }
                if ((tid & 63) == 0) {
                    cursor[4 + (tid >> 6)] = vm;
                    cursor[8 + (tid >> 6)] = vu;
                }
                __syncthreads();
                if (tid == 0) {
                    seg[2048 + 0] = cursor[4] + cursor[5] + cursor[6] + cursor[7];
                    seg[2048 + 1] = cursor[8] + cursor[9] + cursor[10] + cursor[11];
                }
                if (!CH && add_stride) {
                    const long long a0 = (long long)(cursor[4] + cursor[5] + cursor[6] + cursor[7]);
                    const long long runs = (long long)(cursor[8] + cursor[9] + cursor[10] + cursor[11]);
                    long long *const A = reinterpret_cast<long long *>(lds + L::U);
                    long long *const part = reinterpret_cast<long long *>(lds + L::REC);
                    __syncthreads();
                    const u32 k0 = 4 * tid;
                    long long x[4], dl[4], tX = 0;
#pragma unroll
                    for (u32 q = 0; q < 4; q++) {
                        const u32 k = k0 + q;
                        x[q] = k == 0 ? -runs : (k <= add_lag ? (long long)seg[1024 + k] - (long long)seg[k] : 0ll);
                        tX += x[q];
                        dl[q] = tX;
                    }
                    const long long bX = block_exclusive_offset(tX, part, tid);
                    long long tD = 0, ex[4];
#pragma unroll
                    for (u32 q = 0; q < 4; q++) {
                        dl[q] += bX;
                        ex[q] = tD;
                        tD += dl[q];
                    }
                    const long long bD = block_exclusive_offset(tD, part, tid);
#pragma unroll
                    for (u32 q = 0; q < 4; q++) A[k0 + q] = a0 + bD + ex[q];
                    __syncthreads();
                    const SpJobDev &jd = jobs.j[j];
                    unsigned long long *out = reinterpret_cast<unsigned long long *>(jd.out);
                    for (u32 d = tid; d <= add_shift; d += 256) {
                        const int32_t k = add_c - (int32_t)d;
                        const long long v = A[k < 0 ? -k : k];
                        if (v) atomicAdd(&out[(size_t)PMX_ROW_MLEN * add_stride + d], (unsigned long long)v);
                    }
                    if (tid == 0 && a0) atomicAdd(&out[(size_t)PMX_ROW_SCALARS * add_stride + 2], (unsigned long long)a0);
                    __syncthreads();
                }
                cntM = 0;
                cntU = 0;
                seg_written = false;
                leaving = false;
            }
            __syncthreads();
        }
        if (!have_tile) break;

        if (round_lo == 0) {
            cntM += pendM;
            cntU += pendU;
        }
        {
            uint4 *const recs = reinterpret_cast<uint4 *>(lds + L::REC) + (sg.slot << sg.lg_region);
            build_edge_records(lds, recs, sg.slot * 4 * nq, lane_in_slot, G, nq, nr);
            for (u32 q = 0; q < nq; q++) {
                u32 wp[4], wn[4];
#pragma unroll
                for (u32 k = 0; k < 4; k++) {
                    const uint4 rec = recs[q * 4 + k];
                    wp[k] = lds_window(lds, rec.y + sg.l4, rec.x);
                    wn[k] = lds_window(lds, rec.z + sg.l4, rec.x);
                }
                const u32 qq = __builtin_amdgcn_readfirstlane(qc + q);
                add_quad(cP, wp[0], wp[1], wp[2], wp[3], qq);
                add_quad(cN, wn[0], wn[1], wn[2], wn[3], qq);
            }
            qc += nq;
        }

        round_lo += SP_CAP;
        if (round_lo >= n) {
            round_lo = 0;
            if (jn != ji || gnext >= g1) {
                leaving = true;
                leave_job = ji;
            }
            ji = jn;
            g = gnext;
        }
    }
}

template <bool CH, typename JT = SpJobTable>
__global__ void __launch_bounds__(256, CH ? AC_WAVES_CH : AC_WAVES)
k_autocorr_edges(const JT jobs, u32 njobs, u32 total_tiles, u32 tiles_per_wg, u32 lgG, u32 *__restrict__ slab,
                 const unsigned char *__restrict__ tile_flags, const u32 *__restrict__ n_flagged, const u32 *__restrict__ plan = nullptr,
                 u32 add_stride = 0, int32_t add_c = 0, u32 add_shift = 0, u32 add_lag = 0)
{
    if (n_flagged && *n_flagged == 0) return;
    __shared__ __align__(16) u32 lds[AcLds::TOTAL];
    autocorr_edges_body<CH, JT>(lds, blockIdx.x, jobs, njobs, total_tiles, tiles_per_wg, lgG, slab, tile_flags, plan, add_stride, add_c,
                                add_shift, add_lag);
}

struct WinCcArgs {
    u32 total_tiles, tiles_per_wg, lgG;
    int32_t c;
    u32 *slab;
    const unsigned char *tile_flags;
    const u32 *plan;
};
struct WinAcArgs {
    u32 total_tiles, tiles_per_wg, lgG;
    u32 add_shift, add_lag;
    u32 *slab;
    const unsigned char *tile_flags;
    const u32 *plan;
};
template <bool DO_NCC>
__global__ void __launch_bounds__(256, SP_WAVES < AC_WAVES ? SP_WAVES : AC_WAVES)
k_windows_flagged(const SpJobTable jobs_cc, const SpJobTable jobs_ac, u32 njobs, u32 nwg_cc, const WinCcArgs w, const WinAcArgs a,
                  const u32 *__restrict__ n_flagged, u32 add_stride)
{
    const bool cc_half = blockIdx.x < nwg_cc;
    if (n_flagged[cc_half ? 0 : 1] == 0) return;
    constexpr u32 LDS_DWORDS = SpLds<true>::TOTAL > AcLds::TOTAL ? SpLds<true>::TOTAL : AcLds::TOTAL;
    __shared__ __align__(16) u32 lds[LDS_DWORDS];
    if (cc_half)
        cc_sparse_body<true, DO_NCC, false, SpJobTable>(lds, blockIdx.x, jobs_cc, njobs, w.total_tiles, w.tiles_per_wg, w.c, w.lgG, w.slab,
                                                        w.tile_flags, w.plan, add_stride);
    else
        autocorr_edges_body<false, SpJobTable>(lds, blockIdx.x - nwg_cc, jobs_ac, njobs, a.total_tiles, a.tiles_per_wg, a.lgG, a.slab,
                                               a.tile_flags, a.plan, add_stride, w.c, a.add_shift, a.add_lag);
}

#ifndef AP_NQ
#define AP_NQ 4
#endif
#define AP_TBW (AP_NQ * SP_TBW)
#define AP_TB (AP_NQ * SP_TB)
#define AP_CAP 256u
#define AP_MAX_LAGS 8192u
#ifndef AP_WAVES
#define AP_WAVES 5
#endif

struct ApRegs {
    uint4 m[AP_NQ], h;
    u32 below[AP_NQ], hbelow;
};

template <bool GUARD>
__device__ __forceinline__ void ap_fetch(ApRegs &ar, const u32 *__restrict__ M, int64_t d0, uint64_t nbits, u32 tid, u32 nh)
{
#pragma unroll
    for (int q = 0; q < AP_NQ; q++) {
        const int64_t j = d0 + (int64_t)q * SP_TBW + 4 * (int64_t)tid;
        ar.m[q] = ld_quad<GUARD>(M, j, nbits);
        ar.below[q] = GUARD ? ld_dword_guarded(M, j - 1, nbits) : M[j - 1];
    }
    ar.h = make_uint4(0, 0, 0, 0);
    ar.hbelow = 0;
    if (tid < nh) {
        const int64_t jh = d0 + AP_TBW + 4 * (int64_t)tid;
        ar.h = ld_quad<GUARD>(M, jh, nbits);
        ar.hbelow = GUARD ? ld_dword_guarded(M, jh - 1, nbits) : M[jh - 1];
    }
}

__device__ __forceinline__ void ap_fetch_job(ApRegs &ar, const SpJobDev &jb, u32 local_tile, u32 tid, u32 nh)
{
    const int64_t d0 = (int64_t)local_tile * AP_TBW;
    const uint64_t hi = (uint64_t)d0 + AP_TBW + 4 * (uint64_t)nh;
    const bool interior = jb.aligned16 && local_tile > 0 && hi + 2 <= jb.nbits / 32;
    if (interior)
        ap_fetch<false>(ar, jb.M, d0, jb.nbits, tid, nh);
    else
        ap_fetch<true>(ar, jb.M, d0, jb.nbits, tid, nh);
}

__device__ __forceinline__ uint4 edge_words(const uint4 m, u32 below)
{
    return make_uint4(m.x ^ __builtin_amdgcn_alignbit(m.x, below, 31), m.y ^ __builtin_amdgcn_alignbit(m.y, m.x, 31),
                      m.z ^ __builtin_amdgcn_alignbit(m.z, m.y, 31), m.w ^ __builtin_amdgcn_alignbit(m.w, m.z, 31));
}

__device__ __forceinline__ u32 popc4(const uint4 v) { return __popc(v.x) + __popc(v.y) + __popc(v.z) + __popc(v.w); }

__device__ __forceinline__ u32 wave_inclusive_scan(u32 v)
{
    v += (u32)__builtin_amdgcn_update_dpp(0, (int)v, 0x111, 0xf, 0xf, true);
    v += (u32)__builtin_amdgcn_update_dpp(0, (int)v, 0x112, 0xf, 0xf, true);
    v += (u32)__builtin_amdgcn_update_dpp(0, (int)v, 0x114, 0xf, 0xf, true);
    v += (u32)__builtin_amdgcn_update_dpp(0, (int)v, 0x118, 0xf, 0xf, true);
    v += (u32)__builtin_amdgcn_update_dpp(0, (int)v, 0x142, 0xa, 0xf, false);
    v += (u32)__builtin_amdgcn_update_dpp(0, (int)v, 0x143, 0xc, 0xf, false);
    return v;
}

#define PMX_SCAN_STEP(ctl)                                                       \
    "v_add_u32_dpp %0, %0, %0 " ctl "\n\tv_add_u32_dpp %1, %1, %1 " ctl "\n\tv_add_u32_dpp %2, %2, %2 " ctl "\n\t"
#define PMX_SCAN_STEP2(ctl) "v_add_u32_dpp %3, %3, %3 " ctl "\n\tv_add_u32_dpp %4, %4, %4 " ctl "\n\t"
__device__ __forceinline__ void wave_inclusive_scan3(u32 &a, u32 &b, u32 &c)
{
    asm volatile("s_nop 4\n\t" PMX_SCAN_STEP("row_shr:1 row_mask:0xf bank_mask:0xf bound_ctrl:1")
                 PMX_SCAN_STEP("row_shr:2 row_mask:0xf bank_mask:0xf bound_ctrl:1")
                 PMX_SCAN_STEP("row_shr:4 row_mask:0xf bank_mask:0xf bound_ctrl:1")
                 PMX_SCAN_STEP("row_shr:8 row_mask:0xf bank_mask:0xf bound_ctrl:1")
                 PMX_SCAN_STEP("row_bcast:15 row_mask:0xa bank_mask:0xf")
                 PMX_SCAN_STEP("row_bcast:31 row_mask:0xc bank_mask:0xf")
                 : "+v"(a), "+v"(b), "+v"(c));
}
__device__ __forceinline__ void wave_inclusive_scan5(u32 &a, u32 &b, u32 &c, u32 &d, u32 &e)
{
    asm volatile("s_nop 4\n\t" PMX_SCAN_STEP("row_shr:1 row_mask:0xf bank_mask:0xf bound_ctrl:1") PMX_SCAN_STEP2("row_shr:1 row_mask:0xf bank_mask:0xf bound_ctrl:1")
                 PMX_SCAN_STEP("row_shr:2 row_mask:0xf bank_mask:0xf bound_ctrl:1") PMX_SCAN_STEP2("row_shr:2 row_mask:0xf bank_mask:0xf bound_ctrl:1")
                 PMX_SCAN_STEP("row_shr:4 row_mask:0xf bank_mask:0xf bound_ctrl:1") PMX_SCAN_STEP2("row_shr:4 row_mask:0xf bank_mask:0xf bound_ctrl:1")
                 PMX_SCAN_STEP("row_shr:8 row_mask:0xf bank_mask:0xf bound_ctrl:1") PMX_SCAN_STEP2("row_shr:8 row_mask:0xf bank_mask:0xf bound_ctrl:1")
                 PMX_SCAN_STEP("row_bcast:15 row_mask:0xa bank_mask:0xf") PMX_SCAN_STEP2("row_bcast:15 row_mask:0xa bank_mask:0xf")
                 PMX_SCAN_STEP("row_bcast:31 row_mask:0xc bank_mask:0xf") PMX_SCAN_STEP2("row_bcast:31 row_mask:0xc bank_mask:0xf")
                 : "+v"(a), "+v"(b), "+v"(c), "+v"(d), "+v"(e));
}

__device__ __forceinline__ void ap_emit(const uint4 e, const uint4 m, u32 idx, u32 base_bit, u32 *list)
{
    const u64 es[2] = {(u64)e.x | ((u64)e.y << 32), (u64)e.z | ((u64)e.w << 32)};
    const u64 ms[2] = {(u64)m.x | ((u64)m.y << 32), (u64)m.z | ((u64)m.w << 32)};
#pragma unroll
    for (u32 k = 0; k < 2; k++) {
        u64 ww = es[k];
        while (ww) {
            const u32 b = (u32)__builtin_ctzll(ww);
            ww &= ww - 1;
            list[idx] = (base_bit + 64u * k + b) | ((u32)((~ms[k] >> b) & 1ull) << 31);
            idx++;
        }
    }
}

template <typename JT = SpJobTable>
__global__ void __launch_bounds__(256, AP_WAVES)
k_autocorr_pairs(const JT jobs, u32 njobs, u32 total_tiles, u32 tiles_per_wg, u32 max_lag, u32 nl, u32 nh,
                 u32 *__restrict__ slab, unsigned char *__restrict__ tile_flags, u32 *__restrict__ n_flagged)
{
    extern __shared__ __align__(16) u32 ap_lds[];
    u32 *const hP = ap_lds;
    u32 *const hN = ap_lds + nl;
    u32 *const lists = hN + nl;
    u32 *const wtot = lists + 2 * AP_CAP;
    u32 *const misc = wtot + 32;

    const u32 tid = threadIdx.x, lane = tid & 63;
    const u32 wave = __builtin_amdgcn_readfirstlane(tid >> 6);
    const u32 g0 = blockIdx.x * tiles_per_wg;
    const u32 g1 = g0 + tiles_per_wg < total_tiles ? g0 + tiles_per_wg : total_tiles;
    if (g0 >= g1) return;
    for (u32 i = tid; i < 2 * nl; i += 256) ap_lds[i] = 0;

    FIRST_JOB(ji, JT, jobs, njobs, g0)
    u32 jn = ji;
    ApRegs ar;
    ap_fetch_job(ar, jobs.j[ji], g0 - jobs.j[ji].tile0, tid, nh);
    const size_t seg_stride = 2 * (size_t)nl + 16;
    u32 cntM = 0, cntU = 0, par = 0;
    __syncthreads();

    for (u32 g = g0; g < g1; g++) {
        uint4 E[AP_NQ], Eh;
        u32 c[AP_NQ], pendM = 0, pendU = 0;
#pragma unroll
        for (int q = 0; q < AP_NQ; q++) {
            E[q] = edge_words(ar.m[q], ar.below[q]);
            c[q] = popc4(E[q]);
            pendM += popc4(ar.m[q]);
            pendU += (c[q] + (ar.m[q].w >> 31) - (ar.below[q] >> 31)) >> 1;
        }
        Eh = edge_words(ar.h, ar.hbelow);
        const u32 ch = popc4(Eh);
        const u32 s01 = wave_inclusive_scan(c[0] | (c[1] << 16));
        const u32 s23 = AP_NQ > 2 ? wave_inclusive_scan(c[AP_NQ > 2 ? 2 : 0] | (c[AP_NQ > 2 ? 3 : 0] << 16)) : 0u;
        const u32 sh = wave_inclusive_scan(ch);
        u32 *const wt = wtot + par * 16;
        if (lane == 63) {
            wt[wave * 4 + 0] = s01;
            wt[wave * 4 + 1] = s23;
            wt[wave * 4 + 2] = sh;
        }
        __syncthreads();
// ... 232 lines not shown
__device__ __forceinline__ void plan_flagged(const PlanLaunch &pl)
{
    const u32 njobs = pl.njobs, total_tiles = pl.total_tiles, nwg = pl.nwg, raw_lo = pl.raw_lo, raw_hi = pl.raw_hi;
    const u32 flags_per_count = pl.flags_per_count;
    const unsigned char *__restrict__ flags = pl.flags;
    const u32 *__restrict__ n_flagged = pl.n_flagged;
    u32 *__restrict__ plan = pl.plan;
    if (!plan) return;
    const u32 F = *n_flagged * flags_per_count;
    if (F == 0) return;
    __shared__ u32 part[16];
    __shared__ u32 jflag0[SP_MAXJOBS + 1], jtile0[SP_MAXJOBS];
    __shared__ u32 sb[2049];
    __shared__ u32 wl[2048];
    __shared__ u32 se[2048];
    const u32 tid = threadIdx.x;
    if (tid < njobs) {
        jflag0[tid] = pl.flag0[tid];
        jtile0[tid] = pl.tile0[tid];
    }
    if (tid == 0) jflag0[njobs] = 0xffffffffu;
    for (u32 w = tid; w <= nwg; w += 1024) sb[w] = total_tiles;
    __syncthreads();
    u32 running = 0;
    for (u32 f0 = raw_lo & ~15u; f0 < raw_hi; f0 += 1024 * 16) {
        const u32 f = f0 + 16 * tid;
        uint4 q = make_uint4(0, 0, 0, 0);
        if (f < raw_hi) q = *reinterpret_cast<const uint4 *>(flags + f);
        if (f < raw_lo || f + 16 > raw_hi) {
            u32 qq[4] = {q.x, q.y, q.z, q.w};
#pragma unroll
            for (u32 k = 0; k < 16; k++)
                if (f + k < raw_lo || f + k >= raw_hi) qq[k >> 2] &= ~(0xffu << (8 * (k & 3)));
            q = make_uint4(qq[0], qq[1], qq[2], qq[3]);
        }
        const u32 m16 = (((q.x & 0x01010101u) * 0x01020408u) >> 24) | ((((q.y & 0x01010101u) * 0x01020408u) >> 24) << 4) |
                        ((((q.z & 0x01010101u) * 0x01020408u) >> 24) << 8) | ((((q.w & 0x01010101u) * 0x01020408u) >> 24) << 12);
        const u32 cnt = __popc(m16);
        u32 tot;
        const u32 rank = running + plan_block_scan(cnt, part, tid, &tot);
        running += tot;
        if (cnt && F < nwg) {
            u32 m = m16, r = rank;
            while (m) {
                const u32 k = (u32)__builtin_ctz(m);
                m &= m - 1;
                u32 ji = 0;
                while (jflag0[ji + 1] <= f + k) ji++;
                if (r < nwg) sb[r] = jtile0[ji] + (f + k - jflag0[ji]);
                r++;
            }
        } else if (cnt) {
            const u32 w_lo = (u32)(((u64)rank * nwg + F - 1) / F), w_hi = (u32)(((u64)(rank + cnt) * nwg + F - 1) / F);
            u64 prod = (u64)w_lo * F;
            u32 quo = (u32)(prod / nwg), rem = (u32)(prod - (u64)quo * nwg);
            for (u32 w = w_lo; w < w_hi && w < nwg; w++) {
                u32 m = m16;
                for (u32 r = quo - rank; r > 0 && m; r--) m &= m - 1;
                if (m) {
                    const u32 k = (u32)__builtin_ctz(m);
                    u32 ji = 0;
                    while (jflag0[ji + 1] <= f + k) ji++;
                    sb[w] = jtile0[ji] + (f + k - jflag0[ji]);
                }
                u64 nr = (u64)rem + F;
                while (nr >= nwg) {
                    nr -= nwg;
                    quo++;
                }
                rem = (u32)nr;
            }
        }
    }
    __syncthreads();
    if (tid == 0) sb[nwg] = total_tiles;
    __syncthreads();
    u32 nlive = 0;
    for (u32 w0 = 0; w0 < nwg; w0 += 1024) {
        const u32 w = w0 + tid;
        u32 start = 0, end = 0, live = 0;
        if (w < nwg) {
            start = sb[w];
            live = start < sb[w + 1] ? 1u : 0u;
            end = F < nwg ? start + live : sb[w + 1];
            plan[2 * w] = start;
            plan[2 * w + 1] = end;
        }
        u32 tot;
        const u32 idx = nlive + plan_block_scan(live, part, tid, &tot);
        if (live) {
            wl[idx] = w;
            se[idx] = end;
            plan[PLAN_LIST + idx] = w;
        }
        nlive += tot;
    }
    __syncthreads();
    if (tid < njobs) {
        const u32 a = pl.tile0[tid], b = a + pl.ntiles[tid];
        u32 lo = 0, hi = nlive;
        while (lo < hi) {
            const u32 mid = (lo + hi) >> 1;
            if (se[mid] > a) hi = mid;
            else lo = mid + 1;
        }
        const u32 first = lo;
        hi = nlive;
        while (lo < hi) {
            const u32 mid = (lo + hi) >> 1;
            if (sb[wl[mid]] >= b) hi = mid;
            else lo = mid + 1;
        }
        plan[PLAN_JOBWG + 2 * tid] = first;
        plan[PLAN_JOBWG + 2 * tid + 1] = lo;
    }
}

__global__ void __launch_bounds__(1024) k_plan_flagged(const PlanLaunch a, const PlanLaunch b)
{
    if (blockIdx.x == 0) plan_flagged(a);
    else plan_flagged(b);
}

#include "kernels_events.h"


static int launch_autocorr_batch(pmx_ctx *ctx, const pmx_job *jobs, uint32_t njobs, uint32_t max_lag, uint32_t mode, uint32_t read_len,
                                 uint32_t max_shift, uint32_t out_stride, const uint32_t *pre_flag0, const unsigned char *pre_flags,
                                 const u32 *pre_nflagged);

static uint32_t lg_slot_lanes(uint32_t nshifts)
{
    const u32 need = (nshifts + 31) / 32;
    u32 lg = 2;
    while ((1u << lg) < need) lg++;
    return lg;
}

static inline bool is_aligned16(const void *p) { return ((uintptr_t)p & 15u) == 0; }

int pmx_sparse_supported(uint32_t max_shift, uint32_t read_len)
{
    return max_shift >= 3 && max_shift <= 65535 && read_len >= 1 && read_len <= 1024;
}

uint32_t pmx_sparse_max_jobs(void) { return SP_MAXJOBS; }

struct VJob {
    const pmx_job *job;
    u32 d_off, d_n;
    u32 flag0;
    bool ranged;
};

static void fill_plan_launch(PlanLaunch &p, const SpJobTable &tab, u32 n, u32 total, u32 nwg, u32 raw_lo, u32 raw_hi,
                             u32 flags_per_count, const unsigned char *flags, const u32 *n_flagged, u32 *plan)
{
    for (u32 i = 0; i < n; i++) {
        p.flag0[i] = tab.j[i].flag0;
        p.tile0[i] = tab.j[i].tile0;
        p.ntiles[i] = tab.j[i].ntiles;
    }
    p.njobs = n; p.total_tiles = total; p.nwg = nwg; p.raw_lo = raw_lo; p.raw_hi = raw_hi;
    p.flags_per_count = flags_per_count; p.flags = flags; p.n_flagged = n_flagged; p.plan = plan;
}

static void plan_launch(pmx_ctx *ctx, const VJob *vj, uint32_t n, bool autocorr, uint32_t wg_per_cu, SpJobDev *out,
                        uint32_t *total_tiles, uint32_t *tiles_per_wg, uint32_t *nwg, uint64_t tile_bits_override = 0)
{
    uint32_t t = 0;
    for (uint32_t i = 0; i < n; i++) {
        SpJobDev &d = out[i];
        const pmx_job &jb = *vj[i].job;
        const uint64_t bits = jb.nbits + (autocorr ? 1 : 0);
        const uint64_t tile_bits = tile_bits_override ? tile_bits_override : (autocorr ? AC_TB : SP_TB);
        uint64_t nt = (bits + tile_bits - 1) / tile_bits;
        if (nt < 1) nt = 1;
        uint32_t first = 0;
        if (vj[i].ranged && jb.tile_count) {
            first = jb.tile_first;
            nt = jb.tile_count;
        }
        d.F = (const u32 *)jb.d_F;
        d.R = (const u32 *)jb.d_R;
        d.M = (const u32 *)jb.d_M;
        d.nbits = jb.nbits;
        d.tile0 = t;
        d.ntiles = (u32)nt;
        d.aligned16 = autocorr ? is_aligned16(jb.d_M)
                               : (is_aligned16(jb.d_F) && is_aligned16(jb.d_R) && (!jb.d_M || is_aligned16(jb.d_M)));
        d.flags = vj[i].d_off == 0 ? 1u : 0u;
        d.d_off = vj[i].d_off;
        d.d_n = vj[i].d_n;
        d.out = (u64 *)jb.d_out;
        d.out2 = (u64 *)jb.d_out2;
        d.flag0 = vj[i].flag0;
        d.tile_first = first;
        t += (u32)nt;
    }
    uint64_t want = (uint64_t)ctx->num_cus * wg_per_cu;
    if (ctx->debug_max_wg && want > ctx->debug_max_wg) want = ctx->debug_max_wg;
    if (want > t) want = t;
    if (want < 1) want = 1;
    const uint32_t tpw = (uint32_t)((t + want - 1) / want);
    const uint32_t nw = (t + tpw - 1) / tpw;
    for (uint32_t i = 0; i < n; i++) {
        SpJobDev &d = out[i];
        d.wg_first = d.tile0 / tpw;
        d.wg_last = (d.tile0 + d.ntiles - 1) / tpw;
    }
    *total_tiles = t;
    *tiles_per_wg = tpw;
    *nwg = nw;
}

static void plan_launch(pmx_ctx *ctx, const VJob *vj, uint32_t n, bool autocorr, uint32_t wg_per_cu, SpJobTable *tab,
                        uint32_t *total_tiles, uint32_t *tiles_per_wg, uint32_t *nwg, uint64_t tile_bits_override = 0)
{
    plan_launch(ctx, vj, n, autocorr, wg_per_cu, tab->j, total_tiles, tiles_per_wg, nwg, tile_bits_override);
}

static int upload_table(pmx_ctx *ctx, const std::vector<SpJobDev> &v, SpJobTableRef *ref)
{
    const void *d = nullptr;
    int rc = pmx_upload_jobtab(ctx, v.data(), v.size() * sizeof(SpJobDev), &d);
    ref->j = (const SpJobDev *)d;
    return rc;
}
#define SP_MAXJOBS_REF 2048u

static void expand_chunks(const pmx_job *jobs, uint32_t njobs, uint32_t nshifts, std::vector<VJob> &out,
                          const uint32_t *flag0 = nullptr)
{
    for (uint32_t i = 0; i < njobs; i++)
        for (uint32_t off = 0; off < nshifts; off += 1024) {
            VJob v;
            v.ranged = false;
            v.job = &jobs[i];
            v.d_off = off;
            v.d_n = nshifts - off < 1024 ? nshifts - off : 1024;
            v.flag0 = flag0 ? flag0[i] : 0;
            out.push_back(v);
        }
}

static bool events_enabled()
{
    static const bool on = [] {
        const char *e = getenv("PMX_CC_EVENTS");
        return !(e && e[0] == '0');
    }();
    return on;
}

struct EvBigPlan {
    u32 hn, lo, nsg, lds_bytes, wg_per_cu, hi;
    u32 ee_lds;
};

static bool events_big_enabled()
{
    static const bool on = [] {
        const char *e = getenv("PMX_CC_EVENTS_BIG");
        return !(e && e[0] == '0');
    }();
    return on;
}

template <bool HAS_M>
static bool ev_big_plan(uint32_t max_shift, EvBigPlan *p, uint32_t fused_lag = 0)
{
    typedef EvLds<HAS_M, true> L;
    const u32 hn = (max_shift + 1 + 127) / 128 * 128;
    const u32 lo = ((2 * max_shift + 31) / 32 + 3) / 4 * 4;
    u32 hi = EV_HI;
    if (fused_lag) {
        const u32 need = ((fused_lag + 31) / 32 + 2 + 3) / 4 * 4;
        hi = need > EV_HI ? need : EV_HI;
        if (hi > 256u) return false;
    }
    static const int forced = [] {
        const char *e = getenv("PMX_EV_NSG");
        return e ? atoi(e) : 0;
    }();
    const u32 lds_cu = 160u * 1024u;
    u32 best_waves = 0;
    for (u32 nsg = 1; nsg <= 4; nsg *= 2) {
        if (forced && (u32)forced != nsg) continue;
        const u32 bytes = L::total(hn, lo, nsg, hi) * 4 + 16;
        if (bytes > lds_cu) continue;
        u32 per_cu = lds_cu / (bytes + 256);
        if (per_cu * nsg > 4) per_cu = 4 / nsg;
        if (per_cu < 1) continue;
        const u32 waves = per_cu * nsg * 4;
        if (waves > best_waves) {
            best_waves = waves;
            p->hn = hn;
            p->lo = lo;
            p->hi = hi;
            p->nsg = nsg;
            p->lds_bytes = bytes - 16;
            p->wg_per_cu = per_cu;
            p->ee_lds = 0;
        }
    }
    static const bool ee_ok = [] {
        const char *e = getenv("PMX_EV_EE_LDS");
        return !(e && e[0] == '0');
    }();
    if (best_waves && fused_lag && ee_ok) {
        const u32 bytes = p->lds_bytes + 16 + hn * 2;
        u32 per_cu = bytes <= lds_cu ? lds_cu / (bytes + 256) : 0;
        if (per_cu * p->nsg > 4) per_cu = 4 / p->nsg;
        if (per_cu >= p->wg_per_cu) {
            p->lds_bytes = bytes - 16;
            p->ee_lds = 1;
        }
    }
    static const bool dbg = getenv("PMX_DEBUG_PLAN") != nullptr;
    if (dbg && best_waves)
        fprintf(stderr, "[ev_big_plan] max_shift %u fused_lag %u: hn %u lo %u hi %u nsg %u lds %u B x %u per CU, row of lags in LDS: %u\n", max_shift,
                fused_lag, p->hn, p->lo, p->hi, p->nsg, p->lds_bytes, p->wg_per_cu, p->ee_lds);
    return best_waves != 0;
}

#define EV_MAX_DEVICES 64
template <bool HAS_M, bool DO_NCC, bool DO_MLEN, bool DEEP>
static u32 ev_resident_per_cu(pmx_ctx *ctx, u32 built_for)
{
    static int cached[EV_MAX_DEVICES];
    static bool known[EV_MAX_DEVICES];
    const int dev = ctx->device >= 0 && ctx->device < EV_MAX_DEVICES ? ctx->device : -1;
    int n = dev >= 0 && known[dev] ? cached[dev] : -1;
    if (n < 0) {
        auto kern = k_cc_events<HAS_M, DO_NCC, DO_MLEN, 1, false, SpJobTable, DEEP>;
        if (hipOccupancyMaxActiveBlocksPerMultiprocessor(&n, reinterpret_cast<const void *>(kern), 256, 0) != hipSuccess || n < 1) {
            (void)hipGetLastError();
            n = (int)built_for;
        }
        if (dev >= 0) {
            cached[dev] = n;
            known[dev] = true;
        }
    }
    return (u32)n < built_for ? (u32)n : built_for;
}

template <bool HAS_M, bool DO_NCC, u32 NSG, bool DO_MLEN = false>
static int ev_big_launch(pmx_ctx *ctx, const EvBigPlan &pl, const SpJobTableRef &tab, u32 n, u32 total, u32 tpw, u32 nwg, u32 c,
                         u32 max_shift, u32 nhr, unsigned char *d_flags, u32 *d_nflagged, u32 *d_jobstat, u32 fused_lag = 0,
                         unsigned char *d_flags_ac = nullptr)
{
    auto kern = k_cc_events<HAS_M, DO_NCC, DO_MLEN, NSG, true, SpJobTableRef>;
    static bool attr_set[EV_MAX_DEVICES];
    const int dev = ctx->device >= 0 && ctx->device < EV_MAX_DEVICES ? ctx->device : -1;
    if (dev < 0 || !attr_set[dev]) {
        PMX_HIP(hipFuncSetAttribute(reinterpret_cast<const void *>(kern), hipFuncAttributeMaxDynamicSharedMemorySize,
                                    160 * 1024 - 64));
        if (dev >= 0) attr_set[dev] = true;
    }
    hipLaunchKernelGGL(kern, dim3(nwg), dim3(256 * NSG), pl.lds_bytes, ctx->stream, tab, n, total, tpw, c, max_shift, nhr, fused_lag,
                       pl.hn, pl.lo, pl.hi | (DO_MLEN && pl.ee_lds ? 1u << 16 : 0u), ctx->d_slab, d_flags, d_flags_ac ? d_flags_ac : d_flags, d_nflagged,
                       d_jobstat);
    PMX_CHECK_LAUNCH("k_cc_events (max_shift > 1023)");
    return PMX_OK;
}

static int launch_cc_window_chunks(pmx_ctx *ctx, const std::vector<VJob> &vjobs, bool has_m, bool do_ncc, int32_t c,
                                   const ReduceSpec &rs, u32 nr, u32 nz, const unsigned char *d_flags, const u32 *d_nflagged)
{
    const bool behind_events = d_flags != nullptr;
    for (size_t lo = 0; lo < vjobs.size(); lo += SP_MAXJOBS_REF) {
        const uint32_t n = (uint32_t)(vjobs.size() - lo < SP_MAXJOBS_REF ? vjobs.size() - lo : SP_MAXJOBS_REF);
        std::vector<SpJobDev> tab(n);
        memset(tab.data(), 0, n * sizeof(SpJobDev));
        uint32_t total, tpw, nwg;
        plan_launch(ctx, &vjobs[lo], n, false, has_m ? SP_WAVES_CH : SP_WAVES_CH_NCC, tab.data(), &total, &tpw, &nwg);
        const size_t wwords = (size_t)(nwg + n) * SP_SEG_ROWS * 1024 + (size_t)nwg * 4 * 12 * 2 + 64;
        int rc = behind_events ? pmx_ensure_slab_fb(ctx, wwords) : pmx_ensure_slab(ctx, wwords);
        if (rc) return rc;
        u32 *const wslab = behind_events ? ctx->d_slab_fb : ctx->d_slab;
        SpJobTableRef ref;
        rc = upload_table(ctx, tab, &ref);
        if (rc) return rc;
        pmx_timed_launch tl;
        rc = pmx_prof_begin(ctx, PMX_KERNEL_CC_SPARSE, &tl, behind_events);
        if (rc) return rc;
#define SP_LAUNCH(HM, NC)                                                                                                   \
    hipLaunchKernelGGL((k_cc_sparse<HM, NC, true, SpJobTableRef>), dim3(nwg), dim3(256), 0, ctx->stream, ref, n, total, tpw, c, 5u, \
                       wslab, d_flags, d_nflagged, (const u32 *)nullptr)
        if (has_m && do_ncc) SP_LAUNCH(true, true);
        else if (has_m) SP_LAUNCH(true, false);
        else SP_LAUNCH(false, true);
#undef SP_LAUNCH
        PMX_CHECK_LAUNCH("k_cc_sparse");
        rc = pmx_prof_end(ctx, &tl);
        if (rc) return rc;
        hipLaunchKernelGGL(k_reduce_segments<SpJobTableRef>, dim3(behind_events ? 8 : 32, nr + nz, n), dim3(256), 0, ctx->stream,
                           (const u32 *)wslab, ref, (u32)SP_SEG_ROWS, rs, d_nflagged);
        PMX_CHECK_LAUNCH("k_reduce_segments");
    }
    return PMX_OK;
}

static int launch_cc_events_big(pmx_ctx *ctx, const pmx_job *jobs, uint32_t njobs, uint32_t max_shift, uint32_t read_len,
                                bool do_ncc, uint32_t out_stride, const ReduceSpec &rs, u32 nr, u32 nz, uint32_t fused_lag,
                                pmx_fused_mlen *fused)
{
    const bool has_m = jobs[0].d_M != nullptr;
    const u32 c = read_len - 1;
    EvBigPlan pl;
    bool fuse_mlen = has_m && fused && fused_lag && pmx_events_can_fuse_mlen(max_shift, fused_lag) && ev_big_plan<true>(max_shift, &pl, fused_lag);
    if (!fuse_mlen && !(has_m ? ev_big_plan<true>(max_shift, &pl) : ev_big_plan<false>(max_shift, &pl))) {
        pmx_set_error("k_cc_events: no launch geometry for max_shift %u", max_shift);
        return PMX_ERR_INVALID;
    }
    if (fuse_mlen) fused->done = true;
    std::vector<uint32_t> flag0(njobs);
    uint64_t total_flags = 0;
    for (uint32_t i = 0; i < njobs; i++) {
        flag0[i] = (uint32_t)total_flags;
        total_flags += (jobs[i].nbits + SP_TB - 1) / SP_TB + EV_NQ;
    }
    const size_t flag_bytes = (size_t)((total_flags + 15) / 16 * 16);
    const uint32_t per_launch = njobs < SP_MAXJOBS_REF ? njobs : SP_MAXJOBS_REF;
    const size_t stat_bytes = 4 * (size_t)per_launch * sizeof(u32);
    const size_t nflag_arrays = fuse_mlen ? 2 : 1;
    int rc = pmx_ensure_flags_cc(ctx, nflag_arrays * flag_bytes + 16 + stat_bytes);
    if (rc) return rc;
    unsigned char *d_flags = ctx->d_flags_cc;
    unsigned char *d_flags_ac = fuse_mlen ? ctx->d_flags_cc + flag_bytes : nullptr;
    u32 *d_nflagged = (u32 *)(ctx->d_flags_cc + nflag_arrays * flag_bytes);
    u32 *d_jobstat = d_nflagged + 4;
    PMX_HIP(hipMemsetAsync(ctx->d_flags_cc, 0, nflag_arrays * flag_bytes + 16 + stat_bytes, ctx->stream));
    ctx->flags_cc_zeroed[0] = ctx->flags_cc_zeroed[1] = ctx->flags_cc_dirty[0] = ctx->flags_cc_dirty[1] = 0;

    ReduceSpec rs_ev = rs;
    for (u32 i = 0; i < nr; i++)
        if (rs.dst_row[i] == PMX_ROW_MSCC_FSUM || rs.dst_row[i] == PMX_ROW_MSCC_RSUM) rs_ev.is_signed[i] = 1;
    rs_ev.rowlen = pl.hn;
    const u32 nhr = (max_shift + 1 + 127) / 128;
    for (uint32_t lo = 0; lo < njobs; lo += SP_MAXJOBS_REF) {
        const uint32_t n = njobs - lo < SP_MAXJOBS_REF ? njobs - lo : SP_MAXJOBS_REF;
        std::vector<VJob> ev(n);
        for (auto &v : ev) v.ranged = false;
        for (uint32_t i = 0; i < n; i++) {
            ev[i].job = &jobs[lo + i];
            ev[i].d_off = 0;
            ev[i].d_n = max_shift + 1;
            ev[i].flag0 = flag0[lo + i];
        }
        std::vector<SpJobDev> tab(n);
        memset(tab.data(), 0, n * sizeof(SpJobDev));
        uint32_t total, tpw, nwg;
        if (lo) PMX_HIP(hipMemsetAsync(d_jobstat, 0, stat_bytes, ctx->stream));
        plan_launch(ctx, ev.data(), n, false, pl.wg_per_cu, tab.data(), &total, &tpw, &nwg, EV_TB);
        rc = pmx_ensure_slab(ctx, (size_t)(nwg + n) * EV_SEG_ROWS * pl.hn + (size_t)nwg * 4 * pl.nsg * 12 * 2 + 64);
        if (rc) return rc;
        SpJobTableRef ref;
        rc = upload_table(ctx, tab, &ref);
        if (rc) return rc;
        pmx_timed_launch tl;
        rc = pmx_prof_begin(ctx, PMX_KERNEL_CC_EVENTS, &tl);
        if (rc) return rc;
#define EVB(HM, NC, ML)                                                                                                                 \
    (pl.nsg == 1   ? ev_big_launch<HM, NC, 1, ML>(ctx, pl, ref, n, total, tpw, nwg, c, max_shift, nhr, d_flags, d_nflagged, d_jobstat,  \
                                                  ML ? fused_lag : 0u, d_flags_ac)                                                      \
     : pl.nsg == 2 ? ev_big_launch<HM, NC, 2, ML>(ctx, pl, ref, n, total, tpw, nwg, c, max_shift, nhr, d_flags, d_nflagged, d_jobstat,  \
                                                  ML ? fused_lag : 0u, d_flags_ac)                                                      \
                   : ev_big_launch<HM, NC, 4, ML>(ctx, pl, ref, n, total, tpw, nwg, c, max_shift, nhr, d_flags, d_nflagged, d_jobstat,  \
                                                  ML ? fused_lag : 0u, d_flags_ac))
        if (fuse_mlen) rc = do_ncc ? EVB(true, true, true) : EVB(true, false, true);
        else rc = has_m ? (do_ncc ? EVB(true, true, false) : EVB(true, false, false)) : EVB(false, true, false);
#undef EVB
        if (rc) return rc;
        rc = pmx_prof_end(ctx, &tl);
        if (rc) return rc;
        hipLaunchKernelGGL(k_reduce_segments<SpJobTableRef>, dim3(32, nr + nz, n), dim3(256), 0, ctx->stream,
                           (const u32 *)ctx->d_slab, ref, (u32)EV_SEG_ROWS, rs_ev, (const u32 *)nullptr);
        PMX_CHECK_LAUNCH("k_reduce_segments");
        if (fuse_mlen) {
            const u32 lagcap = (u32)(((size_t)fused_lag + 1 + 1023) / 1024 * 1024);
            ReduceSpec r2;
            memset(&r2, 0, sizeof r2);
            r2.nrows = 2;
            r2.src_row[0] = 5; r2.dst_row[0] = 0; r2.is_signed[0] = 1;
            r2.src_row[1] = 4; r2.dst_row[1] = 2 * lagcap; r2.is_scalar[1] = 1; r2.scalar_off = 4;
            r2.nzero = 1;
            r2.zero_row[0] = lagcap;
            r2.use_out2 = 1;
            r2.n_override = fused_lag + 1;
            r2.out_stride = out_stride;
            r2.rowlen = pl.hn;
            hipLaunchKernelGGL(k_reduce_segments<SpJobTableRef>, dim3(32, 3, n), dim3(256), 0, ctx->stream, (const u32 *)ctx->d_slab, ref,
                               (u32)EV_SEG_ROWS, r2, (const u32 *)nullptr);
            PMX_CHECK_LAUNCH("k_reduce_segments (mappable-length pairs)");
        }
        if (has_m) {
            EvTailPlan tp;
            memset(&tp, 0, sizeof tp);
            hipLaunchKernelGGL(k_events_tail<SpJobTableRef>, dim3(n, 1), dim3(EV_TAIL_THREADS), 0, ctx->stream, (const u32 *)ctx->d_slab,
                               ref, tp, (const u32 *)nullptr, (const u32 *)nullptr, (const u32 *)d_nflagged, max_shift, out_stride, 1u,
                               do_ncc ? 1u : 0u, 0u, 1024u, (int32_t)c, 0u, pl.hn, 0u, (const u32 *)nullptr, (const u32 *)nullptr, 0u);
            PMX_CHECK_LAUNCH("k_events_tail");
        }
    }
    std::vector<VJob> vjobs;
    expand_chunks(jobs, njobs, max_shift + 1, vjobs, flag0.data());
    ReduceSpec rs_w = rs;
    rs_w.accumulate = 1;
    rc = launch_cc_window_chunks(ctx, vjobs, has_m, do_ncc, (int32_t)c, rs_w, nr, nz, d_flags, d_nflagged);
    if (rc || !fuse_mlen) return rc;
    return launch_autocorr_batch(ctx, jobs, njobs, fused_lag, 1, read_len, max_shift, out_stride, flag0.data(), d_flags_ac, d_nflagged + 1);
}

uint32_t pmx_cc_batch_jobs(uint32_t max_shift) { return max_shift > 1023 ? SP_MAXJOBS_REF : SP_MAXJOBS; }
uint32_t pmx_autocorr_batch_jobs(void) { return SP_MAXJOBS_REF; }

int pmx_events_take_big(uint32_t max_shift)
{
    return max_shift > 1023 && max_shift <= EV_MAX_SHIFT && events_enabled() && events_big_enabled();
}

int pmx_events_can_fuse_mlen(uint32_t max_shift, uint32_t max_lag)
{
    static const bool fuse = [] {
        const char *e = getenv("PMX_CC_FUSE_MLEN");
        return !(e && e[0] == '0');
    }();
    if (!(events_enabled() && fuse)) return 0;
    if (max_shift <= 1023) return max_lag <= 1023;
    static const bool fuse_big = [] {
        const char *e = getenv("PMX_CC_FUSE_MLEN_BIG");
        return !(e && e[0] == '0');
    }();
    EvBigPlan pl;
    return fuse_big && pmx_events_take_big(max_shift) && ev_big_plan<true>(max_shift, &pl, max_lag);
}

int pmx_events_used(uint32_t max_shift) { return (max_shift <= 1023 && events_enabled()) || pmx_events_take_big(max_shift); }

int pmx_events_big_subgroups(uint32_t max_shift, int has_m)
{
    if (!pmx_events_take_big(max_shift)) return 0;
    EvBigPlan pl;
    if (!(has_m ? ev_big_plan<true>(max_shift, &pl) : ev_big_plan<false>(max_shift, &pl))) return 0;
    return (int)pl.nsg;
}

static int ev_flag_area(pmx_ctx *ctx, size_t area_bytes, size_t zero_bytes, unsigned char **cur, unsigned char **other,
                        size_t *other_dirty)
{
    const size_t half = (area_bytes + 255) & ~(size_t)255;
    const size_t before = ctx->flags_cc_bytes;
    int rc = pmx_ensure_flags_cc(ctx, 2 * half);
    if (rc) return rc;
    if (ctx->flags_cc_bytes != before) ctx->flags_cc_zeroed[0] = ctx->flags_cc_zeroed[1] = ctx->flags_cc_dirty[0] = ctx->flags_cc_dirty[1] = 0;
    const size_t stride = (ctx->flags_cc_bytes / 2) & ~(size_t)255;
    const u32 a = ctx->flags_cc_area & 1u;
    ctx->flags_cc_area = a ^ 1u;
    *cur = ctx->d_flags_cc + a * stride;
    *other = ctx->d_flags_cc + (a ^ 1u) * stride;
    if (ctx->flags_cc_dirty[a]) {
        PMX_HIP(hipMemsetAsync(*cur, 0, ctx->flags_cc_dirty[a], ctx->stream));
        ctx->flags_cc_dirty[a] = 0;
    }
    if (ctx->flags_cc_zeroed[a] < zero_bytes) {
        PMX_HIP(hipMemsetAsync(*cur, 0, zero_bytes, ctx->stream));
        ctx->flags_cc_zeroed[a] = zero_bytes;
    }
    ctx->flags_cc_dirty[a] = zero_bytes;
    *other_dirty = ctx->flags_cc_dirty[a ^ 1u];
    return PMX_OK;
}

int pmx_launch_cc_sparse_batch(pmx_ctx *ctx, const pmx_job *jobs, uint32_t njobs, uint32_t max_shift,
                               uint32_t read_len, bool do_ncc, uint32_t out_stride, bool zero_mlen,
                               uint32_t fused_lag, pmx_fused_mlen *fused)
{
    if (fused) fused->done = false;
    if (njobs == 0) return PMX_OK;
    const bool has_m = jobs[0].d_M != nullptr;
    if (!has_m && !do_ncc) return PMX_OK;
    const bool chunked = max_shift > 1023;
    const int32_t c = (int32_t)read_len - 1;
    const u32 lgG = chunked ? 5u : lg_slot_lanes(max_shift + 1);

    ReduceSpec rs;
    memset(&rs, 0, sizeof rs);
    u32 nr = 0, nz = 0;
    if (do_ncc) { rs.src_row[nr] = 0; rs.dst_row[nr] = PMX_ROW_NCC_CCBINS; nr++; }
    else rs.zero_row[nz++] = PMX_ROW_NCC_CCBINS;
    if (has_m) {
        rs.src_row[nr] = 1; rs.dst_row[nr] = PMX_ROW_MSCC_FSUM; nr++;
        rs.src_row[nr] = 2; rs.dst_row[nr] = PMX_ROW_MSCC_CCBINS; nr++;
        rs.src_row[nr] = 3; rs.dst_row[nr] = PMX_ROW_MSCC_RSUM; nr++;
        if (zero_mlen) rs.zero_row[nz++] = PMX_ROW_MLEN;
    } else {
        rs.zero_row[nz++] = PMX_ROW_MSCC_FSUM;
        rs.zero_row[nz++] = PMX_ROW_MSCC_CCBINS;
        rs.zero_row[nz++] = PMX_ROW_MSCC_RSUM;
        rs.zero_row[nz++] = PMX_ROW_MLEN;
    }
    rs.src_row[nr] = 4; rs.dst_row[nr] = PMX_ROW_SCALARS; rs.is_scalar[nr] = 1; nr++;
    rs.nrows = nr;
    rs.nzero = nz;
    rs.out_stride = out_stride;
    rs.use_out2 = 0;
    rs.keep_scalar2 = (has_m && !zero_mlen) ? 1 : 0;

    if (!ctx->window_only && pmx_events_take_big(max_shift))
        return launch_cc_events_big(ctx, jobs, njobs, max_shift, read_len, do_ncc, out_stride, rs, nr, nz, fused_lag, fused);

    std::vector<VJob> vjobs;
    expand_chunks(jobs, njobs, max_shift + 1, vjobs);
    if (chunked)
        return launch_cc_window_chunks(ctx, vjobs, has_m, do_ncc, c, rs, nr, nz, nullptr, nullptr);

    bool small_vectors = true;
    for (uint32_t i = 0; i < njobs; i++) small_vectors = small_vectors && jobs[i].nbits < (1ull << 32);
    const bool use_events = events_enabled() && !ctx->window_only && !chunked && small_vectors;
    const bool fuse_mlen = use_events && has_m && fused && njobs <= SP_MAXJOBS && pmx_events_can_fuse_mlen(max_shift, fused_lag);
    for (uint32_t i = 0; i < njobs; i++)
        if (jobs[i].tile_count && (!use_events || (has_m && fused && !fuse_mlen))) {
            pmx_set_error("pmx_cc_batch_ranges_dev: tile ranges are taken by the event kernel of max_shift <= 1023 only (not with "
                          "PMX_FLAG_WINDOW_ONLY, PMX_CC_EVENTS=0 or vectors of 2^32 bits)");
            return PMX_ERR_INVALID;
        }
    unsigned char *d_flags = nullptr, *d_flags_ac = nullptr;
    u32 *d_nflagged = nullptr, *d_plan_cc = nullptr, *d_plan_ac = nullptr, *d_jobstat = nullptr;
    size_t flag_bytes_all = 0;
    unsigned char *d_other_area = nullptr;
    size_t other_dirty = 0;
    if (use_events) {
        uint64_t total_flags = 0;
        for (size_t i = 0; i < vjobs.size(); i++) {
            vjobs[i].flag0 = (uint32_t)total_flags;
            total_flags += (vjobs[i].job->nbits + SP_TB - 1) / SP_TB + EV_NQ;
        }
        const size_t flag_bytes = (size_t)((total_flags + 15) / 16 * 16);
        const size_t stat_bytes = EV_STAT_BYTES;
        const size_t zero_bytes = 2 * flag_bytes + 16 + stat_bytes;
        unsigned char *area = nullptr;
        int rc = ev_flag_area(ctx, zero_bytes + 2 * PLAN_WORDS * sizeof(u32), zero_bytes, &area, &d_other_area, &other_dirty);
        if (rc) return rc;
        d_flags = area;
        d_flags_ac = area + flag_bytes;
        d_nflagged = (u32 *)(area + 2 * flag_bytes);
        d_jobstat = (u32 *)(area + 2 * flag_bytes + 16);
        flag_bytes_all = flag_bytes;
        d_plan_cc = (u32 *)((unsigned char *)d_jobstat + stat_bytes);
        d_plan_ac = d_plan_cc + PLAN_WORDS;
        if (fuse_mlen) fused->done = true;
    }
    ReduceSpec rs_ev = rs;
    for (u32 i = 0; i < nr; i++)
        if (rs.dst_row[i] == PMX_ROW_MSCC_FSUM || rs.dst_row[i] == PMX_ROW_MSCC_RSUM) rs_ev.is_signed[i] = 1;

    for (size_t lo = 0; lo < vjobs.size(); lo += SP_MAXJOBS) {
        const uint32_t n = (uint32_t)(vjobs.size() - lo < SP_MAXJOBS ? vjobs.size() - lo : SP_MAXJOBS);
        SpJobTable tab;
        uint32_t total, tpw, nwg;
        int rc;
        pmx_timed_launch tl;
        const u32 raw_lo = use_events ? vjobs[lo].flag0 : 0u;
        const u32 raw_hi = use_events ? (lo + n < vjobs.size() ? vjobs[lo + n].flag0 : (u32)flag_bytes_all) : 0u;
        if (use_events) {
            memset(&tab, 0, sizeof tab);
            if (lo) PMX_HIP(hipMemsetAsync(d_nflagged, 0, 16 + EV_STAT_BYTES, ctx->stream));
            const bool deep = has_m && ctx->deep_lists;
            u32 per_cu = has_m ? (deep ? 4 : EV_WAVES) : EV_WAVES_NCC;
            {
#define EV_OCC(HM, NC, ML, DP) ev_resident_per_cu<HM, NC, ML, DP>(ctx, per_cu)
                if (has_m && do_ncc && fuse_mlen) per_cu = deep ? EV_OCC(true, true, true, true) : EV_OCC(true, true, true, false);
                else if (has_m && do_ncc) per_cu = deep ? EV_OCC(true, true, false, true) : EV_OCC(true, true, false, false);
                else if (has_m && fuse_mlen) per_cu = deep ? EV_OCC(true, false, true, true) : EV_OCC(true, false, true, false);
                else if (has_m) per_cu = deep ? EV_OCC(true, false, false, true) : EV_OCC(true, false, false, false);
                else per_cu = EV_OCC(false, true, false, false);
#undef EV_OCC
            }
            for (uint32_t i = 0; i < n; i++) vjobs[lo + i].ranged = true;
            plan_launch(ctx, &vjobs[lo], n, false, per_cu, &tab, &total, &tpw, &nwg, EV_TB);
            for (uint32_t i = 0; i < n; i++) vjobs[lo + i].ranged = false;
            rc = pmx_ensure_slab(ctx, (size_t)(nwg + n) * EV_SEG_ROWS * 1024 + (size_t)nwg * 4 * 12 * 2 + 64);
            if (rc) return rc;
            rc = pmx_prof_begin(ctx, PMX_KERNEL_CC_EVENTS, &tl);
            if (rc) return rc;
            const u32 nhr = (max_shift + 1 + 127) / 128;
#define EV_LAUNCH_(HM, NC, ML, DP)                                                                                     \
    hipLaunchKernelGGL((k_cc_events<HM, NC, ML, 1, false, SpJobTable, DP>), dim3(nwg), dim3(256), 0, ctx->stream, tab, n, total, tpw, \
                       (u32)c, max_shift, nhr, fused_lag, 1024u, (u32)EV_LO, (u32)EV_HI, ctx->d_slab, d_flags, d_flags_ac, d_nflagged, d_jobstat)
#define EV_LAUNCH(HM, NC, ML)                \
    do {                                     \
        if (deep) EV_LAUNCH_(HM, NC, ML, HM); \
        else EV_LAUNCH_(HM, NC, ML, false);  \
    } while (0)
            if (has_m && do_ncc && fuse_mlen) EV_LAUNCH(true, true, true);
            else if (has_m && do_ncc) EV_LAUNCH(true, true, false);
            else if (has_m && fuse_mlen) EV_LAUNCH(true, false, true);
            else if (has_m) EV_LAUNCH(true, false, false);
            else EV_LAUNCH_(false, true, false, false);
#undef EV_LAUNCH
#undef EV_LAUNCH_
            PMX_CHECK_LAUNCH("k_cc_events");
            rc = pmx_prof_end(ctx, &tl);
            if (rc) return rc;
        }
        SpJobTable tabW, tabA;
        std::vector<VJob> va(n);
        for (auto &v : va) v.ranged = false;
        uint32_t totalA = 0, tpwA = 0, nwgA = 0;
        memset(&tabW, 0, sizeof tabW);
        plan_launch(ctx, &vjobs[lo], n, false, chunked ? (has_m ? SP_WAVES_CH : SP_WAVES_CH_NCC) : (has_m ? SP_WAVES : SP_WAVES_NCC), &tabW, &total, &tpw, &nwg);
        const size_t wwords = (size_t)(nwg + n) * SP_SEG_ROWS * 1024 + (size_t)nwg * 4 * 12 * 2 + 64;
        rc = use_events ? pmx_ensure_slab_fb(ctx, wwords) : pmx_ensure_slab(ctx, wwords);
        if (rc) return rc;
        u32 *const wslab = use_events ? ctx->d_slab_fb : ctx->d_slab;
        if (use_events) {
            if (nwg > 2048) {
                pmx_set_error("k_events_finish: %u workgroups exceed the planner's tables", nwg);
                return PMX_ERR_INVALID;
            }
            PlanLaunch pcc, pac;
            memset(&pcc, 0, sizeof pcc);
            memset(&pac, 0, sizeof pac);
            fill_plan_launch(pcc, tabW, n, total, nwg, raw_lo, raw_hi, (u32)EV_NQ, (const unsigned char *)d_flags, d_nflagged, d_plan_cc);
            if (fuse_mlen) {
                for (uint32_t i = 0; i < n; i++) {
                    va[i].job = vjobs[lo + i].job;
                    va[i].d_off = 0;
                    va[i].d_n = fused_lag + 1;
                    va[i].flag0 = vjobs[lo + i].flag0;
                }
                memset(&tabA, 0, sizeof tabA);
                plan_launch(ctx, va.data(), n, true, AC_WAVES, &tabA, &totalA, &tpwA, &nwgA);
                if (nwgA > 2048) {
                    pmx_set_error("k_events_finish: %u workgroups exceed the planner's tables", nwgA);
                    return PMX_ERR_INVALID;
                }
                fill_plan_launch(pac, tabA, n, totalA, nwgA, raw_lo, raw_hi, 1u, (const unsigned char *)d_flags_ac, d_nflagged + 1, d_plan_ac);
            }
            EvFinishArgs fa;
            memset(&fa, 0, sizeof fa);
            fa.slab = ctx->d_slab;
            fa.jobsum = EV_JOBSUM(d_jobstat);
            fa.S = max_shift;
            fa.out_stride = out_stride;
            fa.has_m = has_m ? 1u : 0u;
            fa.do_ncc = do_ncc ? 1u : 0u;
            fa.fused_mlen = fuse_mlen ? 1u : 0u;
            fa.zero_mlen = zero_mlen ? 1u : 0u;
            fa.keep_scalar2 = rs.keep_scalar2;
            fa.zero_area = reinterpret_cast<uint4 *>(d_other_area);
            fa.zero_quads = (u32)(other_dirty / 16);
            hipLaunchKernelGGL(k_events_finish, dim3(EVF_CHUNKS, EVF_TASKS, n + 1), dim3(1024), 0, ctx->stream, tab, n, fa, pcc, pac);
            PMX_CHECK_LAUNCH("k_events_finish");
            ctx->flags_cc_dirty[(ctx->flags_cc_area & 1u)] = 0;
        }
        if (use_events && fuse_mlen) {
            rc = pmx_ensure_slab_ac(ctx, (size_t)(nwgA + n) * AC_SEG_ROWS * 1024);
            if (rc) return rc;
            rc = pmx_prof_begin(ctx, PMX_KERNEL_CC_SPARSE, &tl, true);
            if (rc) return rc;
            WinCcArgs wa;
            wa.total_tiles = total; wa.tiles_per_wg = tpw; wa.lgG = lgG; wa.c = c;
            wa.slab = wslab; wa.tile_flags = d_flags; wa.plan = d_plan_cc;
            WinAcArgs aa;
            aa.total_tiles = totalA; aa.tiles_per_wg = tpwA; aa.lgG = lg_slot_lanes(fused_lag + 1);
            aa.add_shift = max_shift; aa.add_lag = fused_lag;
            aa.slab = ctx->d_slab_ac; aa.tile_flags = d_flags_ac; aa.plan = d_plan_ac;
            if (do_ncc)
                hipLaunchKernelGGL(k_windows_flagged<true>, dim3(nwg + nwgA), dim3(256), 0, ctx->stream, tabW, tabA, n, nwg, wa, aa,
                                   (const u32 *)d_nflagged, out_stride);
            else
                hipLaunchKernelGGL(k_windows_flagged<false>, dim3(nwg + nwgA), dim3(256), 0, ctx->stream, tabW, tabA, n, nwg, wa, aa,
                                   (const u32 *)d_nflagged, out_stride);
            PMX_CHECK_LAUNCH("k_windows_flagged");
            rc = pmx_prof_end(ctx, &tl);
            if (rc) return rc;
            continue;
        }
        rc = pmx_prof_begin(ctx, PMX_KERNEL_CC_SPARSE, &tl, use_events);
        if (rc) return rc;
#define SP_LAUNCH(HM, NC, CK)                                                                                       \
    hipLaunchKernelGGL((k_cc_sparse<HM, NC, CK>), dim3(nwg), dim3(256), 0, ctx->stream, tabW, n, total, tpw, c, lgG, \
                       wslab, (const unsigned char *)d_flags, (const u32 *)d_nflagged, (const u32 *)(use_events ? d_plan_cc : nullptr), \
                       use_events ? out_stride : 0u)
        if (chunked) {
            if (has_m && do_ncc) SP_LAUNCH(true, true, true);
            else if (has_m) SP_LAUNCH(true, false, true);
            else SP_LAUNCH(false, true, true);
        } else {
            if (has_m && do_ncc) SP_LAUNCH(true, true, false);
            else if (has_m) SP_LAUNCH(true, false, false);
            else SP_LAUNCH(false, true, false);
        }
#undef SP_LAUNCH
        PMX_CHECK_LAUNCH("k_cc_sparse");
        rc = pmx_prof_end(ctx, &tl);
        if (rc) return rc;
        if (!use_events) {
            hipLaunchKernelGGL(k_reduce_segments, dim3(32, nr + nz, n), dim3(256), 0, ctx->stream, (const u32 *)ctx->d_slab, tabW,
                               (u32)SP_SEG_ROWS, rs, (const u32 *)nullptr);
            PMX_CHECK_LAUNCH("k_reduce_segments");
            continue;
        }
    }
    return PMX_OK;
}

size_t pmx_autocorr_scratch_words(uint32_t max_lag)
{
    const size_t lagcap = ((size_t)max_lag + 1 + 1023) / 1024 * 1024;
    return 3 * lagcap + 16;
}

int pmx_launch_autocorr_edges_batch(pmx_ctx *ctx, const pmx_job *jobs, uint32_t njobs, uint32_t max_lag, uint32_t mode,
                                    uint32_t read_len, uint32_t max_shift, uint32_t out_stride)
{
    return launch_autocorr_batch(ctx, jobs, njobs, max_lag, mode, read_len, max_shift, out_stride, nullptr, nullptr, nullptr);
}

static int launch_autocorr_batch(pmx_ctx *ctx, const pmx_job *jobs, uint32_t njobs, uint32_t max_lag, uint32_t mode,
                                 uint32_t read_len, uint32_t max_shift, uint32_t out_stride, const uint32_t *pre_flag0,
                                 const unsigned char *pre_flags, const u32 *pre_nflagged)
{
    if (njobs == 0) return PMX_OK;
    const bool chunked = max_lag > 1023;
    const u32 lagcap = (u32)(((size_t)max_lag + 1 + 1023) / 1024 * 1024);
    const u32 lgG = chunked ? 5u : lg_slot_lanes(max_lag + 1);
    typedef SpJobTableRef JT;

    static const bool pairs_enabled = [] {
        const char *e = getenv("PMX_AUTOCORR_PAIRS");
        return !(e && e[0] == '0');
    }();
    const bool use_pairs = !pre_flags && pairs_enabled && max_lag + 1 <= AP_MAX_LAGS;
    std::vector<uint32_t> flag0(njobs, 0);
    unsigned char *d_flags = const_cast<unsigned char *>(pre_flags);
    u32 *d_nflagged = const_cast<u32 *>(pre_nflagged);
    if (pre_flags)
        for (uint32_t i = 0; i < njobs; i++) flag0[i] = pre_flag0[i];
    const u32 nl = (max_lag + 1 + 63) / 64 * 64;
    int rc;
    if (use_pairs) {
        uint64_t total_flags = 0;
        for (uint32_t i = 0; i < njobs; i++) {
            flag0[i] = (uint32_t)total_flags;
            total_flags += (jobs[i].nbits + 1 + AC_TB - 1) / AC_TB + AP_NQ / AC_NQ;
        }
        const size_t flag_bytes = (size_t)((total_flags + 15) / 16 * 16);
        rc = pmx_ensure_flags(ctx, flag_bytes + 16);
        if (rc) return rc;
        d_flags = ctx->d_flags;
        d_nflagged = (u32 *)(ctx->d_flags + flag_bytes);
        PMX_HIP(hipMemsetAsync(ctx->d_flags, 0, flag_bytes + 16, ctx->stream));
        const u32 nh = (max_lag + 1 + 127) / 128;
        const size_t lds_bytes = (2 * (size_t)nl + 2 * AP_CAP + 32 + 16) * sizeof(u32);
        const size_t seg_stride = 2 * (size_t)nl + 16;
        u32 per_cu = (u32)((160u * 1024u) / (lds_bytes + 512));
        if (per_cu > AP_WAVES) per_cu = AP_WAVES;
        if (per_cu < 1) per_cu = 1;
        for (uint32_t lo = 0; lo < njobs; lo += SP_MAXJOBS_REF) {
            const uint32_t n = njobs - lo < SP_MAXJOBS_REF ? njobs - lo : SP_MAXJOBS_REF;
            std::vector<VJob> vj(n);
            for (auto &v : vj) v.ranged = false;
            for (uint32_t i = 0; i < n; i++) {
                vj[i].job = &jobs[lo + i];
                vj[i].d_off = 0;
                vj[i].d_n = max_lag + 1;
                vj[i].flag0 = flag0[lo + i];
            }
            std::vector<SpJobDev> tab(n);
            memset(tab.data(), 0, n * sizeof(SpJobDev));
            uint32_t total, tpw, nwg;
            plan_launch(ctx, vj.data(), n, true, per_cu, tab.data(), &total, &tpw, &nwg, AP_TB);
            rc = pmx_ensure_slab2(ctx, (size_t)(nwg + n) * seg_stride);
            if (rc) return rc;
            JT ref;
            rc = upload_table(ctx, tab, &ref);
            if (rc) return rc;
            if (lds_bytes > 64 * 1024) {
                static bool attr_set[EV_MAX_DEVICES];
                const int dev = ctx->device >= 0 && ctx->device < EV_MAX_DEVICES ? ctx->device : -1;
                if (dev < 0 || !attr_set[dev]) {
                    PMX_HIP(hipFuncSetAttribute(reinterpret_cast<const void *>(k_autocorr_pairs<JT>),
                                                hipFuncAttributeMaxDynamicSharedMemorySize, 160 * 1024 - 64));
                    if (dev >= 0) attr_set[dev] = true;
                }
            }
            pmx_timed_launch tl;
            rc = pmx_prof_begin(ctx, PMX_KERNEL_AUTOCORR, &tl);
            if (rc) return rc;
            hipLaunchKernelGGL(k_autocorr_pairs<JT>, dim3(nwg), dim3(256), lds_bytes, ctx->stream, ref, n, total, tpw, max_lag, nl,
                               nh, ctx->d_slab2, d_flags, d_nflagged);
            PMX_CHECK_LAUNCH("k_autocorr_pairs");
            rc = pmx_prof_end(ctx, &tl);
            if (rc) return rc;
            hipLaunchKernelGGL(k_reduce_pairs<JT>, dim3((max_lag + 1 + 31) / 32 < 64 ? (max_lag + 1 + 31) / 32 : 64, 3, n), dim3(256), 0,
                               ctx->stream, (const u32 *)ctx->d_slab2, ref, nl, max_lag, lagcap, 0u);
            PMX_CHECK_LAUNCH("k_reduce_pairs");
        }
    }

    std::vector<VJob> vjobs;
    expand_chunks(jobs, njobs, max_lag + 1, vjobs, flag0.data());

    ReduceSpec rs;
    memset(&rs, 0, sizeof rs);
    rs.nrows = 3;
    rs.src_row[0] = 0; rs.dst_row[0] = 0;
    rs.src_row[1] = 1; rs.dst_row[1] = lagcap;
    rs.src_row[2] = 2; rs.dst_row[2] = 2 * lagcap; rs.is_scalar[2] = 1;
    rs.use_out2 = 1;
    rs.accumulate = (use_pairs || pre_flags) ? 1 : 0;
    rs.out_stride = out_stride;

    for (size_t lo = 0; lo < vjobs.size(); lo += SP_MAXJOBS_REF) {
        const uint32_t n = (uint32_t)(vjobs.size() - lo < SP_MAXJOBS_REF ? vjobs.size() - lo : SP_MAXJOBS_REF);
        std::vector<SpJobDev> tab(n);
        memset(tab.data(), 0, n * sizeof(SpJobDev));
        uint32_t total, tpw, nwg;
        plan_launch(ctx, &vjobs[lo], n, true, chunked ? AC_WAVES_CH : AC_WAVES, tab.data(), &total, &tpw, &nwg);
        rc = pmx_ensure_slab_ac(ctx, (size_t)(nwg + n) * AC_SEG_ROWS * 1024);
        if (rc) return rc;
        JT ref;
        rc = upload_table(ctx, tab, &ref);
        if (rc) return rc;
        pmx_timed_launch tl;
        rc = pmx_prof_begin(ctx, PMX_KERNEL_AUTOCORR, &tl);
        if (rc) return rc;
        if (chunked)
            hipLaunchKernelGGL((k_autocorr_edges<true, JT>), dim3(nwg), dim3(256), 0, ctx->stream, ref, n, total, tpw, lgG,
                               ctx->d_slab_ac, (const unsigned char *)d_flags, (const u32 *)d_nflagged, (const u32 *)nullptr);
        else
            hipLaunchKernelGGL((k_autocorr_edges<false, JT>), dim3(nwg), dim3(256), 0, ctx->stream, ref, n, total, tpw, lgG,
                               ctx->d_slab_ac, (const unsigned char *)d_flags, (const u32 *)d_nflagged, (const u32 *)nullptr);
        PMX_CHECK_LAUNCH("k_autocorr_edges");
        rc = pmx_prof_end(ctx, &tl);
        if (rc) return rc;
        hipLaunchKernelGGL(k_reduce_segments<JT>, dim3(32, 3, n), dim3(256), 0, ctx->stream, (const u32 *)ctx->d_slab_ac, ref,
                           (u32)AC_SEG_ROWS, rs, (const u32 *)d_nflagged);
        PMX_CHECK_LAUNCH("k_reduce_segments");
    }
    for (uint32_t lo = 0; lo < njobs; lo += SP_MAXJOBS_REF) {
        const uint32_t n = njobs - lo < SP_MAXJOBS_REF ? njobs - lo : SP_MAXJOBS_REF;
        std::vector<SpJobDev> tab(n);
        memset(tab.data(), 0, n * sizeof(SpJobDev));
        for (uint32_t i = 0; i < n; i++) {
            tab[i].flags = 1;
            tab[i].out = (u64 *)jobs[lo + i].d_out;
            tab[i].out2 = (u64 *)jobs[lo + i].d_out2;
        }
        JT ref;
        rc = upload_table(ctx, tab, &ref);
        if (rc) return rc;
        hipLaunchKernelGGL(k_autocorr_finish<JT>, dim3(n), dim3(AC_FINISH_THREADS), 0, ctx->stream, ref, max_lag, lagcap, mode,
                           (int32_t)read_len - 1, max_shift, out_stride);
        PMX_CHECK_LAUNCH("k_autocorr_finish");
// ... 4 lines not shown
```

Before: 7169000 billion.

## Fuse flagged-window sparse pass into events finish kernel with on-device work sharing

The events kernel now records per-segment flagged-tile counts in the slab and zeroes the output rows itself. The finish kernel then has extra blocks that run the flagged cross-correlation and autocorrelation windows directly. Those blocks split flagged tiles across workgroups with an in-block prefix scan, which removes the separate planner step and the k_windows_flagged launch. Output writes become atomic adds so the fused sparse bodies and the reductions can accumulate into the same rows. This relies on the outputs having been zeroed first, and adds scan overhead to every sparse workgroup.

```diff
diff --git a/pymasc_amd/csrc/kernels_events.h b/pymasc_amd/csrc/kernels_events.h
--- a/pymasc_amd/csrc/kernels_events.h
+++ b/pymasc_amd/csrc/kernels_events.h
@@ -29,6 +29,7 @@
 #define EV_RSENT 0x3fffffffu
 #define EV_JOBSUM(jobstat) (reinterpret_cast<unsigned long long *>((jobstat) + 4 * SP_MAXJOBS))
 #define EV_STAT_BYTES (4 * SP_MAXJOBS * sizeof(u32) + 6 * SP_MAXJOBS * sizeof(unsigned long long))
+#define EV_COUNTS_AT(segment) (((size_t)(segment) * EV_SEG_ROWS + 4) * 1024 + 6)
 #define EV_SEG_ROWS 6u
 #define EV_MAX_SHIFT 8191u
 #ifndef EV_PRIO_STAGE
@@ -269,7 +270,8 @@
 __global__ void __launch_bounds__(256 * NSG, BIG ? 4 : (HAS_M ? (DEEP ? 4 : EV_WAVES) : EV_WAVES_NCC))
 k_cc_events(const JT jobs, u32 njobs, u32 total_tiles, u32 tiles_per_wg, u32 c, u32 S, u32 nhr, u32 max_lag,
             u32 hn_arg, u32 lo_arg, u32 hi_arg, u32 *__restrict__ slab, unsigned char *__restrict__ tile_flags,
-            unsigned char *__restrict__ tile_flags_ac, u32 *__restrict__ n_flagged, u32 *__restrict__ jobstat)
+            unsigned char *__restrict__ tile_flags_ac, u32 *__restrict__ n_flagged, u32 *__restrict__ jobstat, u32 zstride = 0,
+            u32 zmask = 0)
 {
     typedef EvLds<HAS_M, BIG, DEEP> L;
     static_assert(!DEEP || (HAS_M && !BIG), "DEEP: the max_shift <= 1023 instantiations with a track");
@@ -303,6 +305,23 @@
     const u32 g0 = blockIdx.x * tiles_per_wg;
     const u32 g1 = g0 + tiles_per_wg < total_tiles ? g0 + tiles_per_wg : total_tiles;
     if (g0 >= g1) return;
+    if (!BIG && zmask) {
+        const u32 ncol = S + 1, per_job = (u32)__popc(zmask & 31u) * ncol + 3u, cells = njobs * per_job;
+        const u32 share = (cells + gridDim.x - 1) / gridDim.x;
+        const u32 z0 = blockIdx.x * share, z1 = z0 + share < cells ? z0 + share : cells;
+        for (u32 i = z0 + gt; i < z1; i += NT) {
+            const u32 job = i / per_job, r = i - job * per_job;
+            u64 *const out = jobs.j[job].out;
+            if (r < 3) {
+                if (r < 2 || (zmask & 32u)) out[(size_t)PMX_ROW_SCALARS * zstride + r] = 0;
+            } else {
+                const u32 rr = (r - 3) / ncol, col = (r - 3) - rr * ncol;
+                u32 m = zmask & 31u;
+                for (u32 k = 0; k < rr; k++) m &= m - 1;
+                out[(size_t)__builtin_ctz(m) * zstride + col] = 0;
+            }
+        }
+    }
     {
 #pragma nounroll
         for (u32 i = gt; i < L::o_sg(HN); i += NT) lds[i] = 0;
@@ -783,6 +802,7 @@
                                         : (accF + L::POOL > 32767u || (DO_MLEN && accE + EV_CAPE(BIG) > 32767u)));
         if (NSG == 1 && leaving && tid == 0) {
             const u32 pc = xch[14], pa = xch[15];
+            if (!BIG) *reinterpret_cast<uint2 *>(slab + EV_COUNTS_AT(blockIdx.x + ji)) = make_uint2(pc, pa);
             if (pc) atomicAdd(n_flagged, pc);
             if (pa) atomicAdd(n_flagged + 1, pa);
             xch[14] = 0;
@@ -1021,28 +1041,140 @@
 
 #define EVF_TASKS 6u
 #define EVF_CHUNKS 8u
+#define EVF_ZBLOCKS 32u
 struct EvFinishArgs {
     const u32 *slab;
     const unsigned long long *jobsum;
     u32 S, out_stride, has_m, do_ncc, fused_mlen, zero_mlen, keep_scalar2;
     uint4 *zero_area;
     u32 zero_quads;
+    const u32 *n_flagged;
+    u32 nwg_cc, nwg_ac;
 };
-
-__global__ void __launch_bounds__(1024)
-k_events_finish(const SpJobTable jobs, u32 njobs, const EvFinishArgs a, const PlanLaunch pcc, const PlanLaunch pac)
+struct EvShareTab {
+    u32 wg_first[SP_MAXJOBS], wg_last[SP_MAXJOBS], tile0[SP_MAXJOBS], ntiles[SP_MAXJOBS], tile_first[SP_MAXJOBS];
+    u32 tiles_per_wg, nseg;
+    const u32 *slab;
+};
+
+template <u32 FPC, u32 WHICH>
+__device__ __forceinline__ uint2 ev_flagged_share(u32 *const sh, const EvShareTab &es, const SpJobTable &wj, u32 njobs, u32 total_tiles,
+                                                  u32 nwg, u32 w, u32 counted, const unsigned char *__restrict__ flags)
 {
-    __shared__ u32 acc[128];
-    const u32 tid = threadIdx.x, chunk = blockIdx.x, task = blockIdx.y, job = blockIdx.z;
-    if (job == njobs) {
-        const u32 id = task * EVF_CHUNKS + chunk, nid = EVF_TASKS * EVF_CHUNKS;
-        if (id == 0) plan_flagged(pcc);
-        else if (id == 1) plan_flagged(pac);
-        else
-            for (u32 i = (id - 2) * 1024 + tid; i < a.zero_quads; i += (nid - 2) * 1024) a.zero_area[i] = make_uint4(0, 0, 0, 0);
+    const u32 tid = threadIdx.x, lane = tid & 63u;
+    const u64 F = (u64)counted * FPC;
+    const bool few = F < nwg;
+    if (few && w >= F) return make_uint2(0u, 0u);
+    const u64 rank[2] = {few ? (u64)w : (u64)w * F / nwg, few ? (u64)w + 1 : (w + 1 == nwg ? F : (u64)(w + 1) * F / nwg)};
+    const u32 N = es.nseg, K = (N + 255u) / 256u;
+    const u32 i0 = tid * K < N ? tid * K : N, i1 = i0 + K < N ? i0 + K : N;
+    u32 mine = 0;
+    for (u32 j = 0; j < njobs; j++) {
+        const u32 lo = es.wg_first[j] + j, hi = es.wg_last[j] + j + 1;
+        for (u32 i = i0 > lo ? i0 : lo; i < (i1 < hi ? i1 : hi); i++) mine += es.slab[EV_COUNTS_AT(i) + WHICH];
+    }
+    u32 x = mine;
+    for (int off = 1; off < 64; off <<= 1) {
+        const u32 y = __shfl_up(x, off, 64);
+        if (lane >= (u32)off) x += y;
+    }
+    if (lane == 63) sh[tid >> 6] = x;
+    if (tid < 4) sh[4 + tid] = 0xffffffffu;
+    __syncthreads();
+    u32 base = x - mine;
+    for (u32 v = 0; v < (tid >> 6); v++) base += sh[v];
+#pragma unroll
+    for (u32 e = 0; e < 2; e++) {
+        const u64 q = rank[e] / FPC;
+        if (q >= base && q < (u64)base + mine) {
+            u32 before = base;
+            for (u32 j = 0; j < njobs; j++) {
+                const u32 lo = es.wg_first[j] + j, hi = es.wg_last[j] + j + 1;
+                for (u32 i = i0 > lo ? i0 : lo; i < (i1 < hi ? i1 : hi); i++) {
+                    const u32 cnt = es.slab[EV_COUNTS_AT(i) + WHICH];
+                    if (q >= before && q < (u64)before + cnt) {
+                        sh[4 + 2 * e] = i;
+                        sh[5 + 2 * e] = (u32)q - before;
+                    }
+                    before += cnt;
+                }
+            }
+        }
+    }
+    __syncthreads();
+    u32 res[2];
+#pragma unroll
+    for (u32 e = 0; e < 2; e++) {
+        const u32 i = sh[4 + 2 * e];
+        u32 o = sh[5 + 2 * e];
+        res[e] = total_tiles;
+        if (i < N) {
+            u32 j = 0;
+            while (j + 1 < njobs && es.wg_first[j + 1] + j + 1 <= i) j++;
+            const u32 b = i - j;
+            const u32 jt0 = es.tile0[j], jt1 = jt0 + es.ntiles[j];
+            const u32 t0 = b * es.tiles_per_wg > jt0 ? b * es.tiles_per_wg : jt0;
+            const u32 t1 = (b + 1) * es.tiles_per_wg < jt1 ? (b + 1) * es.tiles_per_wg : jt1;
+            const unsigned char *__restrict__ fl = flags + wj.j[j].flag0;
+            u32 found = t1;
+            for (u32 t = t0; t < t1 && b <= es.wg_last[j]; t += 64) {
+                const u32 lt = t + lane - jt0 + es.tile_first[j];
+                const bool set = t + lane < t1 && fl[(size_t)FPC * lt] != 0;
+                unsigned long long m = __ballot(set);
+                const u32 c = (u32)__popcll(m);
+                if (o < c) {
+                    for (; o > 0; o--) m &= m - 1;
+                    found = t + (u32)__builtin_ctzll(m);
+                    break;
+                }
+                o -= c;
+            }
+            const u32 widx = FPC * (found - jt0 + es.tile_first[j]) + (u32)(rank[e] % FPC);
+            const u32 wn = wj.j[j].ntiles;
+            res[e] = wj.j[j].tile0 + (widx < wn ? widx : wn);
+        }
+        res[e] = res[e] < total_tiles ? res[e] : total_tiles;
+    }
+    __syncthreads();
+    if (few) res[1] = res[0] < res[1] ? res[0] + 1 : res[0];
+    return make_uint2(res[0], res[1]);
+}
+
+template <bool HAS_M, bool DO_NCC, bool AC>
+__global__ void __launch_bounds__(256, AC ? (SP_WAVES < AC_WAVES ? SP_WAVES : AC_WAVES) : (HAS_M ? SP_WAVES : SP_WAVES_NCC))
+k_events_finish(const SpJobTable jobs_cc, const SpJobTable jobs_ac, u32 njobs, const EvFinishArgs a, const EvShareTab es,
+                const WinCcArgs wc, const WinAcArgs wa)
+{
+    constexpr u32 LDS_DWORDS = AC && AcLds::TOTAL > SpLds<HAS_M>::TOTAL ? AcLds::TOTAL : SpLds<HAS_M>::TOTAL;
+    __shared__ __align__(16) u32 lds[LDS_DWORDS];
+    static_assert(LDS_DWORDS >= 128, "the sum blocks keep 128 columns in LDS");
+    const u32 tid = threadIdx.x, nfin = EVF_CHUNKS * EVF_TASKS * njobs;
+    if (blockIdx.x >= nfin) {
+        u32 bx = blockIdx.x - nfin;
+        if (bx < EVF_ZBLOCKS) {
+            for (u32 i = bx * 256 + tid; i < a.zero_quads; i += EVF_ZBLOCKS * 256) a.zero_area[i] = make_uint4(0, 0, 0, 0);
+            return;
+        }
+        bx -= EVF_ZBLOCKS;
+        if (bx < a.nwg_cc) {
+            const u32 counted = a.n_flagged[0];
+            if (counted == 0) return;
+            const uint2 r = ev_flagged_share<EV_NQ, 0>(lds, es, jobs_cc, njobs, wc.total_tiles, a.nwg_cc, bx, counted, wc.tile_flags);
+            cc_sparse_body<HAS_M, DO_NCC, false, SpJobTable>(lds, bx, jobs_cc, njobs, wc.total_tiles, wc.tiles_per_wg, wc.c, wc.lgG, wc.slab,
+                                                             wc.tile_flags, nullptr, a.out_stride, true, r.x, r.y);
+        } else if (AC) {
+            bx -= a.nwg_cc;
+            const u32 counted = a.n_flagged[1];
+            if (counted == 0 || bx >= a.nwg_ac) return;
+            const uint2 r = ev_flagged_share<1, 1>(lds, es, jobs_ac, njobs, wa.total_tiles, a.nwg_ac, bx, counted, wa.tile_flags);
+            autocorr_edges_body<false, SpJobTable>(lds, bx, jobs_ac, njobs, wa.total_tiles, wa.tiles_per_wg, wa.lgG, wa.slab, wa.tile_flags,
+                                                   nullptr, a.out_stride, wc.c, wa.add_shift, wa.add_lag, true, r.x, r.y);
+        }
         return;
     }
-    const SpJobDev &jb = jobs.j[job];
+    u32 *const acc = lds;
+    const u32 chunk = blockIdx.x % EVF_CHUNKS, task = (blockIdx.x / EVF_CHUNKS) % EVF_TASKS, job = blockIdx.x / (EVF_CHUNKS * EVF_TASKS);
+    const SpJobDev &jb = jobs_cc.j[job];
     const u32 S = a.S, n = S + 1;
     u64 *const out = jb.out;
     const size_t os = a.out_stride;
@@ -1050,9 +1182,11 @@
     if (task == 0) {
         if (chunk != 0) return;
         u64 *dst = out + (size_t)PMX_ROW_SCALARS * os;
-        for (u32 k = tid; k < a.out_stride; k += 1024) {
-            if (k == 2 && a.keep_scalar2 && !a.fused_mlen) continue;
-            dst[k] = k < 2 ? js[k] : (k == 2 ? (a.fused_mlen ? js[4] : 0ull) : (k == 3 && jb.tile_first == 0 ? (u64)PMX_PATH_SPARSE : 0ull));
+        for (u32 k = tid; k < a.out_stride; k += 256) {
+            if (k < 2) atomicAdd(&dst[k], js[k]);
+            else if (k == 2 && a.fused_mlen) atomicAdd(&dst[k], js[4]);
+            else if (k == 2 && a.keep_scalar2) continue;
+            else dst[k] = k == 3 && es.tile_first[job] == 0 ? (u64)PMX_PATH_SPARSE : 0ull;
         }
         return;
     }
@@ -1063,9 +1197,9 @@
     u64 *dst = out + (size_t)dst_row * os;
     if (!produced) {
         if (task != 5 || !a.has_m || a.zero_mlen)
-            for (u32 k = col0 + tid; k < a.out_stride && k < col0 + 128; k += 1024) dst[k] = 0;
+            for (u32 k = col0 + tid; k < a.out_stride && k < col0 + 128; k += 256) dst[k] = 0;
         if (chunk == EVF_CHUNKS - 1 && (task != 5 || !a.has_m || a.zero_mlen))
-            for (u32 k = 128 * EVF_CHUNKS + tid; k < a.out_stride; k += 1024) dst[k] = 0;
+            for (u32 k = 128 * EVF_CHUNKS + tid; k < a.out_stride; k += 256) dst[k] = 0;
         return;
     }
     if (col0 >= n) return;
@@ -1075,13 +1209,20 @@
     const u32 q = tid & 31u, g = tid >> 5;
     const size_t stride = (size_t)EV_SEG_ROWS * 1024;
     const u32 *p = a.slab + (size_t)job * stride + (size_t)src_row * 1024 + col0 + 4 * q;
+    const u32 wl = es.wg_last[job];
     u32 s0 = 0, s1 = 0, s2 = 0, s3 = 0;
-    for (u32 w = jb.wg_first + g; w <= jb.wg_last; w += 32) {
-        const uint4 v = *reinterpret_cast<const uint4 *>(p + (size_t)w * stride);
-        s0 += v.x;
-        s1 += v.y;
-        s2 += v.z;
-        s3 += v.w;
+    for (u32 w = es.wg_first[job] + g; w <= wl; w += 32) {
+        uint4 v[4];
+#pragma unroll
+        for (u32 k = 0; k < 4; k++)
+            v[k] = w + 8 * k <= wl ? *reinterpret_cast<const uint4 *>(p + (size_t)(w + 8 * k) * stride) : make_uint4(0, 0, 0, 0);
+#pragma unroll
+        for (u32 k = 0; k < 4; k++) {
+            s0 += v[k].x;
+            s1 += v[k].y;
+            s2 += v[k].z;
+            s3 += v[k].w;
+        }
     }
     atomicAdd(&acc[4 * q + 0], s0);
     atomicAdd(&acc[4 * q + 1], s1);
@@ -1090,7 +1231,7 @@
     __syncthreads();
     if (tid < 128 && col0 + tid < n) {
         const u32 t = acc[tid];
-        dst[col0 + tid] = task == 3 ? (u64)(u32)((u32)js[2] - t) : task == 4 ? (u64)(u32)((u32)js[3] + t) : (u64)t;
+        atomicAdd(&dst[col0 + tid], task == 3 ? (u64)(u32)((u32)js[2] - t) : task == 4 ? (u64)(u32)((u32)js[3] + t) : (u64)t);
     }
 }
 
diff --git a/pymasc_amd/csrc/kernels_sparse.hip b/pymasc_amd/csrc/kernels_sparse.hip
--- a/pymasc_amd/csrc/kernels_sparse.hip
+++ b/pymasc_amd/csrc/kernels_sparse.hip
@@ -579,7 +579,8 @@
 template <bool HAS_M, bool DO_NCC, bool CH, typename JT>
 __device__ __forceinline__ void cc_sparse_body(u32 *const lds, const u32 bx, const JT &jobs, u32 njobs, u32 total_tiles, u32 tiles_per_wg,
                                                int32_t c, u32 lgG, u32 *__restrict__ slab, const unsigned char *__restrict__ tile_flags,
-                                               const u32 *__restrict__ plan, u32 add_stride)
+                                               const u32 *__restrict__ plan, u32 add_stride, bool own_range = false, u32 own_g0 = 0,
+                                               u32 own_g1 = 0)
 {
     typedef SpLds<HAS_M> L;
     u32 *const cursor = lds + L::MISC;
@@ -589,8 +590,8 @@
     const u32 tid = threadIdx.x;
     const SlotGeom sg = slot_geom(lgG, tid);
 
-    const u32 g0 = plan ? plan[2 * bx] : bx * tiles_per_wg;
-    const u32 g1 = plan ? plan[2 * bx + 1] : (g0 + tiles_per_wg < total_tiles ? g0 + tiles_per_wg : total_tiles);
+    const u32 g0 = own_range ? own_g0 : plan ? plan[2 * bx] : bx * tiles_per_wg;
+    const u32 g1 = own_range ? own_g1 : plan ? plan[2 * bx + 1] : (g0 + tiles_per_wg < total_tiles ? g0 + tiles_per_wg : total_tiles);
     if (g0 >= g1) return;
 
     for (u32 i = tid; i < 40; i += 256) lds[L::ZERO + i] = 0;
@@ -1211,7 +1212,8 @@
 template <bool CH, typename JT>
 __device__ __forceinline__ void autocorr_edges_body(u32 *const lds, const u32 bx, const JT &jobs, u32 njobs, u32 total_tiles, u32 tiles_per_wg,
                                                     u32 lgG, u32 *__restrict__ slab, const unsigned char *__restrict__ tile_flags,
-                                                    const u32 *__restrict__ plan, u32 add_stride, int32_t add_c, u32 add_shift, u32 add_lag)
+                                                    const u32 *__restrict__ plan, u32 add_stride, int32_t add_c, u32 add_shift, u32 add_lag,
+                                                    bool own_range = false, u32 own_g0 = 0, u32 own_g1 = 0)
 {
     typedef AcLds L;
     u32 *const cursor = lds + L::MISC;
@@ -1221,8 +1223,8 @@
     const u32 tid = threadIdx.x;
     const SlotGeom sg = slot_geom(lgG, tid);
 
-    const u32 g0 = plan ? plan[2 * bx] : bx * tiles_per_wg;
-    const u32 g1 = plan ? plan[2 * bx + 1] : (g0 + tiles_per_wg < total_tiles ? g0 + tiles_per_wg : total_tiles);
+    const u32 g0 = own_range ? own_g0 : plan ? plan[2 * bx] : bx * tiles_per_wg;
+    const u32 g1 = own_range ? own_g1 : plan ? plan[2 * bx + 1] : (g0 + tiles_per_wg < total_tiles ? g0 + tiles_per_wg : total_tiles);
     if (g0 >= g1) return;
 
     for (u32 i = tid; i < 40; i += 256) lds[L::ZERO + i] = 0;
@@ -1446,32 +1448,13 @@
     int32_t c;
     u32 *slab;
     const unsigned char *tile_flags;
-    const u32 *plan;
 };
 struct WinAcArgs {
     u32 total_tiles, tiles_per_wg, lgG;
     u32 add_shift, add_lag;
     u32 *slab;
     const unsigned char *tile_flags;
-    const u32 *plan;
 };
-template <bool DO_NCC>
-__global__ void __launch_bounds__(256, SP_WAVES < AC_WAVES ? SP_WAVES : AC_WAVES)
-k_windows_flagged(const SpJobTable jobs_cc, const SpJobTable jobs_ac, u32 njobs, u32 nwg_cc, const WinCcArgs w, const WinAcArgs a,
-                  const u32 *__restrict__ n_flagged, u32 add_stride)
-{
-    const bool cc_half = blockIdx.x < nwg_cc;
-    if (n_flagged[cc_half ? 0 : 1] == 0) return;
-    constexpr u32 LDS_DWORDS = SpLds<true>::TOTAL > AcLds::TOTAL ? SpLds<true>::TOTAL : AcLds::TOTAL;
-    __shared__ __align__(16) u32 lds[LDS_DWORDS];
-    if (cc_half)
-        cc_sparse_body<true, DO_NCC, false, SpJobTable>(lds, blockIdx.x, jobs_cc, njobs, w.total_tiles, w.tiles_per_wg, w.c, w.lgG, w.slab,
-                                                        w.tile_flags, w.plan, add_stride);
-    else
-        autocorr_edges_body<false, SpJobTable>(lds, blockIdx.x - nwg_cc, jobs_ac, njobs, a.total_tiles, a.tiles_per_wg, a.lgG, a.slab,
-                                               a.tile_flags, a.plan, add_stride, w.c, a.add_shift, a.add_lag);
-}
-
 #ifndef AP_NQ
 #define AP_NQ 4
 #endif
@@ -2010,18 +1993,6 @@
     u32 flag0;
     bool ranged;
 };
-
-static void fill_plan_launch(PlanLaunch &p, const SpJobTable &tab, u32 n, u32 total, u32 nwg, u32 raw_lo, u32 raw_hi,
-                             u32 flags_per_count, const unsigned char *flags, const u32 *n_flagged, u32 *plan)
-{
-    for (u32 i = 0; i < n; i++) {
-        p.flag0[i] = tab.j[i].flag0;
-        p.tile0[i] = tab.j[i].tile0;
-        p.ntiles[i] = tab.j[i].ntiles;
-    }
-    p.njobs = n; p.total_tiles = total; p.nwg = nwg; p.raw_lo = raw_lo; p.raw_hi = raw_hi;
-    p.flags_per_count = flags_per_count; p.flags = flags; p.n_flagged = n_flagged; p.plan = plan;
-}
 
 static void plan_launch(pmx_ctx *ctx, const VJob *vj, uint32_t n, bool autocorr, uint32_t wg_per_cu, SpJobDev *out,
                         uint32_t *total_tiles, uint32_t *tiles_per_wg, uint32_t *nwg, uint64_t tile_bits_override = 0)
@@ -2219,7 +2190,7 @@
     }
     hipLaunchKernelGGL(kern, dim3(nwg), dim3(256 * NSG), pl.lds_bytes, ctx->stream, tab, n, total, tpw, c, max_shift, nhr, fused_lag,
                        pl.hn, pl.lo, pl.hi | (DO_MLEN && pl.ee_lds ? 1u << 16 : 0u), ctx->d_slab, d_flags, d_flags_ac ? d_flags_ac : d_flags, d_nflagged,
-                       d_jobstat);
+                       d_jobstat, 0u, 0u);
     PMX_CHECK_LAUNCH("k_cc_events (max_shift > 1023)");
     return PMX_OK;
 }
@@ -2486,8 +2457,7 @@
             return PMX_ERR_INVALID;
         }
     unsigned char *d_flags = nullptr, *d_flags_ac = nullptr;
-    u32 *d_nflagged = nullptr, *d_plan_cc = nullptr, *d_plan_ac = nullptr, *d_jobstat = nullptr;
-    size_t flag_bytes_all = 0;
+    u32 *d_nflagged = nullptr, *d_jobstat = nullptr;
     unsigned char *d_other_area = nullptr;
     size_t other_dirty = 0;
     if (use_events) {
@@ -2500,15 +2470,12 @@
         const size_t stat_bytes = EV_STAT_BYTES;
         const size_t zero_bytes = 2 * flag_bytes + 16 + stat_bytes;
         unsigned char *area = nullptr;
-        int rc = ev_flag_area(ctx, zero_bytes + 2 * PLAN_WORDS * sizeof(u32), zero_bytes, &area, &d_other_area, &other_dirty);
+        int rc = ev_flag_area(ctx, zero_bytes, zero_bytes, &area, &d_other_area, &other_dirty);
         if (rc) return rc;
         d_flags = area;
         d_flags_ac = area + flag_bytes;
         d_nflagged = (u32 *)(area + 2 * flag_bytes);
         d_jobstat = (u32 *)(area + 2 * flag_bytes + 16);
-        flag_bytes_all = flag_bytes;
-        d_plan_cc = (u32 *)((unsigned char *)d_jobstat + stat_bytes);
-        d_plan_ac = d_plan_cc + PLAN_WORDS;
         if (fuse_mlen) fused->done = true;
     }
     ReduceSpec rs_ev = rs;
@@ -2518,11 +2485,9 @@
     for (size_t lo = 0; lo < vjobs.size(); lo += SP_MAXJOBS) {
         const uint32_t n = (uint32_t)(vjobs.size() - lo < SP_MAXJOBS ? vjobs.size() - lo : SP_MAXJOBS);
         SpJobTable tab;
-        uint32_t total, tpw, nwg;
+        uint32_t total = 0, tpw = 0, nwg = 0;
         int rc;
         pmx_timed_launch tl;
-        const u32 raw_lo = use_events ? vjobs[lo].flag0 : 0u;
-        const u32 raw_hi = use_events ? (lo + n < vjobs.size() ? vjobs[lo + n].flag0 : (u32)flag_bytes_all) : 0u;
         if (use_events) {
             memset(&tab, 0, sizeof tab);
             if (lo) PMX_HIP(hipMemsetAsync(d_nflagged, 0, 16 + EV_STAT_BYTES, ctx->stream));
@@ -2545,9 +2510,13 @@
             rc = pmx_prof_begin(ctx, PMX_KERNEL_CC_EVENTS, &tl);
             if (rc) return rc;
             const u32 nhr = (max_shift + 1 + 127) / 128;
+            const u32 zmask = (do_ncc ? 1u << PMX_ROW_NCC_CCBINS : 0u) |
+                              (has_m ? (1u << PMX_ROW_MSCC_FSUM | 1u << PMX_ROW_MSCC_RSUM | 1u << PMX_ROW_MSCC_CCBINS) : 0u) |
+                              (fuse_mlen ? (1u << PMX_ROW_MLEN | 32u) : 0u);
 #define EV_LAUNCH_(HM, NC, ML, DP)                                                                                     \
     hipLaunchKernelGGL((k_cc_events<HM, NC, ML, 1, false, SpJobTable, DP>), dim3(nwg), dim3(256), 0, ctx->stream, tab, n, total, tpw, \
-                       (u32)c, max_shift, nhr, fused_lag, 1024u, (u32)EV_LO, (u32)EV_HI, ctx->d_slab, d_flags, d_flags_ac, d_nflagged, d_jobstat)
+                       (u32)c, max_shift, nhr, fused_lag, 1024u, (u32)EV_LO, (u32)EV_HI, ctx->d_slab, d_flags, d_flags_ac, d_nflagged, d_jobstat, \
+                       out_stride, zmask)
 #define EV_LAUNCH(HM, NC, ML)                \
     do {                                     \
         if (deep) EV_LAUNCH_(HM, NC, ML, HM); \
@@ -2565,38 +2534,28 @@
             if (rc) return rc;
         }
         SpJobTable tabW, tabA;
-        std::vector<VJob> va(n);
-        for (auto &v : va) v.ranged = false;
-        uint32_t totalA = 0, tpwA = 0, nwgA = 0;
+        const uint32_t tpw_ev = tpw, nwg_ev = nwg;
         memset(&tabW, 0, sizeof tabW);
-        plan_launch(ctx, &vjobs[lo], n, false, chunked ? (has_m ? SP_WAVES_CH : SP_WAVES_CH_NCC) : (has_m ? SP_WAVES : SP_WAVES_NCC), &tabW, &total, &tpw, &nwg);
+        memset(&tabA, 0, sizeof tabA);
+        plan_launch(ctx, &vjobs[lo], n, false, has_m ? SP_WAVES : SP_WAVES_NCC, &tabW, &total, &tpw, &nwg);
         const size_t wwords = (size_t)(nwg + n) * SP_SEG_ROWS * 1024 + (size_t)nwg * 4 * 12 * 2 + 64;
         rc = use_events ? pmx_ensure_slab_fb(ctx, wwords) : pmx_ensure_slab(ctx, wwords);
         if (rc) return rc;
         u32 *const wslab = use_events ? ctx->d_slab_fb : ctx->d_slab;
         if (use_events) {
-            if (nwg > 2048) {
-                pmx_set_error("k_events_finish: %u workgroups exceed the planner's tables", nwg);
-                return PMX_ERR_INVALID;
-            }
-            PlanLaunch pcc, pac;
-            memset(&pcc, 0, sizeof pcc);
-            memset(&pac, 0, sizeof pac);
-            fill_plan_launch(pcc, tabW, n, total, nwg, raw_lo, raw_hi, (u32)EV_NQ, (const unsigned char *)d_flags, d_nflagged, d_plan_cc);
+            uint32_t totalA = 0, tpwA = 0, nwgA = 0;
             if (fuse_mlen) {
+                std::vector<VJob> va(n);
                 for (uint32_t i = 0; i < n; i++) {
+                    va[i].ranged = false;
                     va[i].job = vjobs[lo + i].job;
                     va[i].d_off = 0;
                     va[i].d_n = fused_lag + 1;
                     va[i].flag0 = vjobs[lo + i].flag0;
                 }
-                memset(&tabA, 0, sizeof tabA);
                 plan_launch(ctx, va.data(), n, true, AC_WAVES, &tabA, &totalA, &tpwA, &nwgA);
-                if (nwgA > 2048) {
-                    pmx_set_error("k_events_finish: %u workgroups exceed the planner's tables", nwgA);
-                    return PMX_ERR_INVALID;
-                }
-                fill_plan_launch(pac, tabA, n, totalA, nwgA, raw_lo, raw_hi, 1u, (const unsigned char *)d_flags_ac, d_nflagged + 1, d_plan_ac);
+                rc = pmx_ensure_slab_ac(ctx, (size_t)(nwgA + n) * AC_SEG_ROWS * 1024);
+                if (rc) return rc;
             }
             EvFinishArgs fa;
             memset(&fa, 0, sizeof fa);
@@ -2611,58 +2570,61 @@
             fa.keep_scalar2 = rs.keep_scalar2;
             fa.zero_area = reinterpret_cast<uint4 *>(d_other_area);
             fa.zero_quads = (u32)(other_dirty / 16);
-            hipLaunchKernelGGL(k_events_finish, dim3(EVF_CHUNKS, EVF_TASKS, n + 1), dim3(1024), 0, ctx->stream, tab, n, fa, pcc, pac);
+            fa.n_flagged = d_nflagged;
+            fa.nwg_cc = nwg;
+            fa.nwg_ac = nwgA;
+            EvShareTab es;
+            memset(&es, 0, sizeof es);
+            for (uint32_t i = 0; i < n; i++) {
+                es.wg_first[i] = tab.j[i].wg_first;
+                es.wg_last[i] = tab.j[i].wg_last;
+                es.tile0[i] = tab.j[i].tile0;
+                es.ntiles[i] = tab.j[i].ntiles;
+                es.tile_first[i] = tab.j[i].tile_first;
+            }
+            es.tiles_per_wg = tpw_ev;
+            es.nseg = nwg_ev + n;
+            es.slab = ctx->d_slab;
+            WinCcArgs wa;
+            wa.total_tiles = total; wa.tiles_per_wg = tpw; wa.lgG = lgG; wa.c = c;
+            wa.slab = wslab; wa.tile_flags = d_flags;
+            WinAcArgs aa;
+            memset(&aa, 0, sizeof aa);
+            aa.total_tiles = totalA; aa.tiles_per_wg = tpwA; aa.lgG = lg_slot_lanes(fused_lag + 1);
+            aa.add_shift = max_shift; aa.add_lag = fused_lag;
+            aa.slab = ctx->d_slab_ac; aa.tile_flags = d_flags_ac;
+            rc = pmx_prof_begin(ctx, PMX_KERNEL_CC_SPARSE, &tl, true);
+            if (rc) return rc;
+            const dim3 grid(EVF_CHUNKS * EVF_TASKS * n + EVF_ZBLOCKS + nwg + nwgA);
+#define EVF_LAUNCH(HM, NC, AC) \
+    hipLaunchKernelGGL((k_events_finish<HM, NC, AC>), grid, dim3(256), 0, ctx->stream, tabW, tabA, n, fa, es, wa, aa)
+            if (has_m && do_ncc && fuse_mlen) EVF_LAUNCH(true, true, true);
+            else if (has_m && fuse_mlen) EVF_LAUNCH(true, false, true);
+            else if (has_m && do_ncc) EVF_LAUNCH(true, true, false);
+            else if (has_m) EVF_LAUNCH(true, false, false);
+            else EVF_LAUNCH(false, true, false);
+#undef EVF_LAUNCH
             PMX_CHECK_LAUNCH("k_events_finish");
             ctx->flags_cc_dirty[(ctx->flags_cc_area & 1u)] = 0;
-        }
-        if (use_events && fuse_mlen) {
-            rc = pmx_ensure_slab_ac(ctx, (size_t)(nwgA + n) * AC_SEG_ROWS * 1024);
-            if (rc) return rc;
-            rc = pmx_prof_begin(ctx, PMX_KERNEL_CC_SPARSE, &tl, true);
-            if (rc) return rc;
-            WinCcArgs wa;
-            wa.total_tiles = total; wa.tiles_per_wg = tpw; wa.lgG = lgG; wa.c = c;
-            wa.slab = wslab; wa.tile_flags = d_flags; wa.plan = d_plan_cc;
-            WinAcArgs aa;
-            aa.total_tiles = totalA; aa.tiles_per_wg = tpwA; aa.lgG = lg_slot_lanes(fused_lag + 1);
-            aa.add_shift = max_shift; aa.add_lag = fused_lag;
-            aa.slab = ctx->d_slab_ac; aa.tile_flags = d_flags_ac; aa.plan = d_plan_ac;
-            if (do_ncc)
-                hipLaunchKernelGGL(k_windows_flagged<true>, dim3(nwg + nwgA), dim3(256), 0, ctx->stream, tabW, tabA, n, nwg, wa, aa,
-                                   (const u32 *)d_nflagged, out_stride);
-            else
-                hipLaunchKernelGGL(k_windows_flagged<false>, dim3(nwg + nwgA), dim3(256), 0, ctx->stream, tabW, tabA, n, nwg, wa, aa,
-                                   (const u32 *)d_nflagged, out_stride);
-            PMX_CHECK_LAUNCH("k_windows_flagged");
             rc = pmx_prof_end(ctx, &tl);
             if (rc) return rc;
             continue;
         }
-        rc = pmx_prof_begin(ctx, PMX_KERNEL_CC_SPARSE, &tl, use_events);
+        rc = pmx_prof_begin(ctx, PMX_KERNEL_CC_SPARSE, &tl);
         if (rc) return rc;
-#define SP_LAUNCH(HM, NC, CK)                                                                                       \
-    hipLaunchKernelGGL((k_cc_sparse<HM, NC, CK>), dim3(nwg), dim3(256), 0, ctx->stream, tabW, n, total, tpw, c, lgG, \
-                       wslab, (const unsigned char *)d_flags, (const u32 *)d_nflagged, (const u32 *)(use_events ? d_plan_cc : nullptr), \
-                       use_events ? out_stride : 0u)
-        if (chunked) {
-            if (has_m && do_ncc) SP_LAUNCH(true, true, true);
-            else if (has_m) SP_LAUNCH(true, false, true);
-            else SP_LAUNCH(false, true, true);
-        } else {
-            if (has_m && do_ncc) SP_LAUNCH(true, true, false);
-            else if (has_m) SP_LAUNCH(true, false, false);
-            else SP_LAUNCH(false, true, false);
-        }
+#define SP_LAUNCH(HM, NC)                                                                                                  \
+    hipLaunchKernelGGL((k_cc_sparse<HM, NC, false>), dim3(nwg), dim3(256), 0, ctx->stream, tabW, n, total, tpw, c, lgG, wslab, \
+                       (const unsigned char *)nullptr, (const u32 *)nullptr, (const u32 *)nullptr, 0u)
+        if (has_m && do_ncc) SP_LAUNCH(true, true);
+        else if (has_m) SP_LAUNCH(true, false);
+        else SP_LAUNCH(false, true);
 #undef SP_LAUNCH
         PMX_CHECK_LAUNCH("k_cc_sparse");
         rc = pmx_prof_end(ctx, &tl);
         if (rc) return rc;
-        if (!use_events) {
-            hipLaunchKernelGGL(k_reduce_segments, dim3(32, nr + nz, n), dim3(256), 0, ctx->stream, (const u32 *)ctx->d_slab, tabW,
-                               (u32)SP_SEG_ROWS, rs, (const u32 *)nullptr);
-            PMX_CHECK_LAUNCH("k_reduce_segments");
-            continue;
-        }
+        hipLaunchKernelGGL(k_reduce_segments, dim3(32, nr + nz, n), dim3(256), 0, ctx->stream, (const u32 *)ctx->d_slab, tabW,
+                           (u32)SP_SEG_ROWS, rs, (const u32 *)nullptr);
+        PMX_CHECK_LAUNCH("k_reduce_segments");
     }
     return PMX_OK;
 }
```

Measured after the change: 7225000 billion, median of 2. Within noise of the previous version (+0.8%).
